# One-2-3-45/One-2-3-45

Measured on NVIDIA H100. Metric: sec/mesh end-to-end (256x256 in), lower is better.
Workload: dtype f16

## Files before the change

### include/o2345.h

```cpp
#ifndef O2345_H_
#define O2345_H_

#include <stddef.h>
#include <stdint.h>

#ifdef __cplusplus
extern "C" {
#endif

#define O2345_OK 0
#define O2345_EINVAL (-1)
#define O2345_ECUDA (-2)
#define O2345_EUNSUPPORTED (-3)

#define O2345_ABI_VERSION 5

typedef void* o2345_stream_t;

int o2345_abi_version(void);
int o2345_last_error(char* buf, size_t n);
int o2345_device_info(int* major, int* minor, int* sms);


#define O2345_SDF_PE 39
#define O2345_SDF_HID 128
#define O2345_SDF_LAT 16
#define O2345_SDF_IN1 144
#define O2345_SDF_PACK_FLOATS (39 * 128 + 128 + 2 * (144 * 128 + 128) + 128 * 144 + 128 * 48)

int o2345_sdf_pack_weights(const float* w0, const float* b0, const float* w1, const float* b1,
                           const float* w2, const float* b2, float* pack, o2345_stream_t stream);

#define O2345_PTS_EXPLICIT 0
#define O2345_PTS_LATTICE 1
#define O2345_PTS_RAYS 2

typedef struct o2345_points {
  int mode;
  const float* pts;
  const float* lin;
  int R;
  const float* rays_o;
  const float* rays_d;
  const float* z;
  int S;
  int z_stride;
} o2345_points;

#define O2345_SDF_FP32 0
#define O2345_SDF_TC_SPLIT 1
int o2345_sdf_query(const o2345_points* src, int64_t n, const float* vol_cl, int D, const float* wpack,
                    const uint8_t* active, float inactive_sdf, int negate, int precision, float* sdf, float* feat,
                    float* latent, float* grad, o2345_stream_t stream);


int o2345_frustum_mask(const float* proj, int V, const float* origin, float voxel_size, int D, int sizeH,
                       int sizeW, int min_views, uint32_t* mask_bits, uint8_t* keep, o2345_stream_t stream);

int64_t o2345_compact_scratch_ints(int64_t n);
int o2345_compact(const uint8_t* flags, int64_t n, int32_t* rows, int32_t* index, int32_t* count,
                  int32_t* scratch, o2345_stream_t stream);

int o2345_costvol_gather(const float* feats_nhwc, int V, int h, int w, int sizeH, int sizeW, const float* proj,
                         const float* origin, float voxel_size, int D, const int32_t* rows, const int32_t* count,
                         int64_t max_rows, const uint32_t* mask_bits, float* cost, o2345_stream_t stream);

int o2345_dense_scatter(const float* feat, const int32_t* rows, const int32_t* count, int64_t max_rows, int D,
                        float* vol_cl, float* vol_cf, float* occ, o2345_stream_t stream);

int o2345_occ_nearest(const o2345_points* src, int64_t n, const float* occ, int D, uint8_t* out,
                      o2345_stream_t stream);


int o2345_sdf_voxels(const float* occ, const float* vol_cl, int D, const float* origin, float voxel_size,
                     const float* wpack, int precision, float* sdf_vol, o2345_stream_t stream);

int o2345_prune_by_sdf(const float* sdf, const float* occ, int D, const float* ladder, int n_ladder, float* scratch,
                       float* minabs, int32_t* counts, o2345_stream_t stream);
int o2345_prune_select(const float* minabs, int64_t n, float threshold, uint8_t* keep, o2345_stream_t stream);
int o2345_clear_flags(const int32_t* rows, const int32_t* idx, int64_t n, uint8_t* flags, o2345_stream_t stream);
int o2345_gather_rows(const int32_t* rows, int64_t n, int D, const float* vol_cf, int C, float* coords, float* feats,
                      o2345_stream_t stream);

int o2345_lod_children(const float* pre_coords, int64_t n, int D1, const uint8_t* frustum_keep, uint8_t* keep,
                       int32_t* parent, int32_t* err_scratch, o2345_stream_t stream);

int o2345_costvol_gather_lod(const float* feats_nhwc, int C, int V, int h, int w, int sizeH, int sizeW, const float* proj,
                             const float* origin, float voxel_size, int D, const int32_t* rows, const int32_t* count,
                             int64_t max_rows, const uint32_t* mask_bits, const int32_t* parent, const float* pre_feats,
                             float* cost, o2345_stream_t stream);


int o2345_sp_coarsen(const int32_t* fine_index, int Ef, const int32_t* fine_rows, const int32_t* fine_count,
                     int64_t max_fine, int Ec, uint8_t* coarse_flags, int32_t* cmin_scratch,
                     o2345_stream_t stream);

int o2345_sp_conv(const float* in_feats, const int32_t* in_index, int Ein, const int32_t* out_rows,
                  const int32_t* out_count, int64_t max_out, int Eout, int mode, const float* kernel, int Cin,
                  int Cout, float* out_raw, double* stats, o2345_stream_t stream);

int o2345_sp_bn_relu(const float* x, const int32_t* count, int64_t max_rows, int C, const double* stats,
                     const float* gamma, const float* beta, float eps, const float* skip, float* out,
                     o2345_stream_t stream);

int o2345_mc_classify(const float* u, int R, float iso, uint8_t* cases, uint8_t* cell_flags, uint8_t* edge_flags,
                      o2345_stream_t stream);
int o2345_mc_vertices(const float* u, int R, float iso, const int32_t* edges, const int32_t* count,
                      int64_t max_verts, double* verts, o2345_stream_t stream);
int64_t o2345_scan_scratch_ints(int64_t n);
int o2345_mc_tri_offsets(const uint8_t* cases, const int32_t* cells, const int32_t* count, int64_t max_cells,
                         const uint8_t* n_tri_table, int32_t* offsets, int32_t* total, int32_t* scratch,
                         o2345_stream_t stream);
int o2345_mc_triangles(const uint8_t* cases, int R, const int32_t* cells, const int32_t* count, int64_t max_cells,
                       const int32_t* tri_offsets, const int8_t* tri_table, const uint8_t* n_tri_table,
                       const int8_t* edge_owner, const int32_t* vert_index, int32_t* tris, o2345_stream_t stream);

typedef struct o2345_view4 {
  float* ptr;
  int64_t sn, sc, sh, sw;
  int c0;
} o2345_view4;

int o2345_conv2d(const float* in, int N, int Cin, int H, int W, const float* weight, const float* bias, int Cout,
                 int K, int stride, int pad, float* out, double* stats, o2345_stream_t stream);
int o2345_abn_apply(const float* x, int N, int C, int H, int W, const double* stats, const float* gamma,
                    const float* beta, float eps, float slope, const o2345_view4* out, o2345_stream_t stream);
int o2345_upsample_bilinear(const float* x, int N, int C, int H, int W, int factor, const float* add,
                            const o2345_view4* out, o2345_stream_t stream);


int o2345_ray_upsample(const float* rays_o, const float* rays_d, int64_t R, const float* z, const float* sdf,
                       int S, float inv_s, const float* occ, int D, const float* u, int n_new, float* new_z,
                       o2345_stream_t stream);
int o2345_ray_merge(const float* z, const float* sdf, int S, const float* new_z, const float* new_sdf, int n_new,
                    int64_t R, float* out_z, float* out_sdf, o2345_stream_t stream);
int o2345_ray_midpoints(const float* rays_o, const float* rays_d, int64_t R, const float* z, int S,
                        float sample_dist, const float* occ, int D, float* mid_z, float* dists, uint8_t* active,
                        o2345_stream_t stream);

#define O2345_MAP_CH 60
#define O2345_RNET_PACK_FLOATS 19664

typedef struct o2345_views {
  int V, H, W;
  const float* maps;
  const float* proj;
  const float* centers;
  float sizeW, sizeH;
} o2345_views;

#define O2345_BLEND_FP32 0
#define O2345_BLEND_TC_FP16 1
int o2345_render_blend(const o2345_points* src, int64_t n, const uint8_t* active, const float* vol_cl,
                       const float* occ, int D, const o2345_views* views, int dir_mode, const float* query_center,
                       const float* dirs, const float* rnet_pack, int precision, float* rgb, int32_t* nvalid,
                       o2345_stream_t stream);

int o2345_ray_composite(const float* rays_d, int64_t R, int S, const float* mid_z, const float* dists,
                        const float* sdf, const float* grad, const float* color, const uint8_t* active,
                        const int32_t* nvalid, float inv_s, float alpha_inter_ratio, int has_background,
                        float background, float* color_out, float* depth_out, float* weights_out, float* cdf_out,
                        float* alpha_out, float* weights_sum_out, uint8_t* color_mask_out, o2345_stream_t stream);

typedef struct {
  const float* bias;
  const void* residual;
  const void* rowbias;
  int64_t rowbias_ld;
  int rows_per_group;
  int act;
  float alpha;
  int out_f32;
  float* colstats;
  int stats_rows_per_group;
} o2345_epilogue;

int o2345_gemm_f16(const void* A, const void* B, void* C, int M, int N, int K, int64_t lda, int64_t ldb,
                   int64_t ldc, int nh, int nb, int64_t stride_a_h, int64_t stride_a_b, int64_t stride_b_h,
                   int64_t stride_b_b, int64_t stride_c_h, int64_t stride_c_b, const o2345_epilogue* ep ,
                   float* splitk_ws, int64_t ws_floats, o2345_stream_t stream);

int o2345_last_trap(char* buf, size_t n);

void o2345_debug_gemm_force(int ctas, int bn, int splits);
void o2345_debug_gemm_persist(int mode, int min_tiles);
void o2345_debug_gemm_model(const float* seven);

void o2345_debug_gemm_trace(long long* device_buf16);

int o2345_conv3x3_f16(const void* x, int B, int H, int W, int C, const void* weight, int N, void* out, int64_t ldc,
                      const o2345_epilogue* ep, float* splitk_ws, int64_t ws_floats, o2345_stream_t stream);

int o2345_conv_up2x_f16(const void* x, int B, int H, int W, int C, const void* weight4, int N, void* out, int64_t ldc,
                        const o2345_epilogue* ep, float* splitk_ws, int64_t ws_floats, o2345_stream_t stream);

int64_t o2345_groupnorm_scratch_floats(int B, int G);
int o2345_groupnorm_stats(const void* x, int B, int HW, int C, int G, float eps, const float* gamma, const float* beta,
                          float* scratch, float* scale, float* shift, o2345_stream_t stream);
int o2345_groupnorm_apply(const void* x, int B, int HW, int C, int G, float eps, const float* gamma, const float* beta, int act,
                          void* out, o2345_stream_t stream);
void o2345_debug_groupnorm_cluster(int cl);
int o2345_norm_act_im2col(const void* x, int B, int H, int W, int C, int ksize, int stride, int upsample, int pad_lo,
                          const float* scale, const float* shift, int act, void* out, o2345_stream_t stream);
int o2345_norm_act_im2col_stats(const void* x, int B, int H, int W, int C, int ksize, int stride, int upsample, int pad_lo,
                                const float* stats_a, int Ca, const float* stats_b, int G, float eps, const float* gamma,
                                const float* beta, int act, void* out, o2345_stream_t stream);
int o2345_layernorm_rows(const void* x, int64_t M, int C, float eps, const float* gamma, const float* beta, void* y,
                         o2345_stream_t stream);
int o2345_softmax_rows(const void* s, int64_t rows, int n, void* p, o2345_stream_t stream);
int o2345_attention_f16(const void* q, const void* k, const void* v, int B, int N, int H, int d, int ld, void* out,
                        int ldo, float scale, o2345_stream_t stream);
int o2345_geglu(const void* x, int64_t M, int I, void* y, o2345_stream_t stream);
int o2345_silu(const void* x, int64_t n, void* y, o2345_stream_t stream);
int o2345_transpose_tokens(const void* x, int B, int N, int C, void* y, o2345_stream_t stream);
int o2345_timestep_embedding(const float* t, int B, int dim, void* out, o2345_stream_t stream);
int o2345_add_channel_bias(void* y, const void* e, int B, int HW, int C, int lde, o2345_stream_t stream);
int o2345_copy_channels(const void* src, int64_t M, int C, void* dst, int ldd, int off, o2345_stream_t stream);
int o2345_nchw_f32_to_cl_f16(const float* x, int B, int C, int HW, void* y, int ldy, int off, o2345_stream_t stream);
int o2345_cl_f16_to_nchw_f32(const void* x, int B, int C, int HW, int ldx, float* y, o2345_stream_t stream);
int o2345_cfg_ddim_update(const float* x, const float* eps, const float* noise, int64_t n, float scale, float a_t,
                          float a_prev, float sigma_t, float sqrt_one_minus_at, float* x_prev, float* pred_x0,
                          o2345_stream_t stream);

int o2345_clip_patches(const float* x, int B, int H, int W, int res, int patch, const float* mean3, const float* std3, int kp,
                       void* out, o2345_stream_t stream);
int o2345_clip_add_positions(void* tok, const float* cls, const float* pos, int B, int N, int d, o2345_stream_t stream);

#ifdef __cplusplus
}
#endif
#endif
```

### one-2-3-45_b200/csrc/gemm_tc.cu

```cuda
#include <cuda.h>
#include <stdlib.h>
#include <cuda_fp16.h>

#include "common.cuh"
#include "wgmma.cuh"

namespace o2345 {
namespace {

constexpr int BM = 128, BK = 64;
constexpr int EPI_WARPS = 8;
constexpr int EPI_THREADS = 32 * EPI_WARPS;
constexpr int GEMM_THREADS = 128 + EPI_THREADS;
constexpr uint64_t WAIT_LIMIT_NS = 4000000000ull;
constexpr int MAX_CLUSTER = 8;
constexpr int RES_PREFETCH = 8;

enum { WAIT_EMPTY = 1, WAIT_FULL = 2 };

struct TrapRecord {
  unsigned long long magic;
  int tag, stage, bx, by, bz, rank, M, N, K, bn, mode, splits, conv;
};
constexpr unsigned long long TRAP_MAGIC = 0x6f32333435545250ull;

__device__ __forceinline__ uint32_t smem_u32(const void* p) { return (uint32_t)__cvta_generic_to_shared(p); }

__device__ __forceinline__ void mbar_init(uint64_t* bar, uint32_t count) {
  asm volatile("mbarrier.init.shared::cta.b64 [%0], %1;" ::"r"(smem_u32(bar)), "r"(count));
}
__device__ __forceinline__ void mbar_expect_tx(uint64_t* bar, uint32_t bytes) {
  asm volatile("mbarrier.arrive.expect_tx.shared::cta.b64 _, [%0], %1;" ::"r"(smem_u32(bar)), "r"(bytes) : "memory");
}
__device__ __forceinline__ void mbar_arrive(uint64_t* bar) {
  asm volatile("mbarrier.arrive.shared::cta.b64 _, [%0];" ::"r"(smem_u32(bar)) : "memory");
}
__device__ __forceinline__ uint32_t mbar_try(uint64_t* bar, uint32_t parity) {
  uint32_t done;
  asm volatile(
      "{\n\t.reg .pred p;\n\t"
      "mbarrier.try_wait.parity.shared::cta.b64 p, [%1], %2;\n\t"
      "selp.u32 %0, 1, 0, p;\n\t}"
      : "=r"(done)
      : "r"(smem_u32(bar)), "r"(parity)
      : "memory");
  return done;
}
__device__ __forceinline__ uint64_t global_ns() {
  uint64_t t;
  asm volatile("mov.u64 %0, %%globaltimer;" : "=l"(t));
  return t;
}
__device__ __forceinline__ void tma_load_2d(void* dst, const CUtensorMap* map, uint64_t* bar, int c0, int c1) {
  asm volatile(
      "cp.async.bulk.tensor.2d.shared::cluster.global.mbarrier::complete_tx::bytes [%0], [%1, {%3, %4}], [%2];"
      ::"r"(smem_u32(dst)), "l"(map), "r"(smem_u32(bar)), "r"(c0), "r"(c1)
      : "memory");
}
__device__ __forceinline__ void tma_load_4d(void* dst, const CUtensorMap* map, uint64_t* bar, int c0, int c1, int c2, int c3) {
  asm volatile(
      "cp.async.bulk.tensor.4d.shared::cluster.global.mbarrier::complete_tx::bytes [%0], [%1, {%3, %4, %5, %6}], [%2];"
      ::"r"(smem_u32(dst)), "l"(map), "r"(smem_u32(bar)), "r"(c0), "r"(c1), "r"(c2), "r"(c3)
      : "memory");
}
__device__ __forceinline__ uint32_t cluster_ctarank() {
  uint32_t r;
  asm volatile("mov.u32 %0, %%cluster_ctarank;" : "=r"(r));
  return r;
}
__device__ __forceinline__ void cluster_sync_all() {
  asm volatile("barrier.cluster.arrive.release.aligned;\n\tbarrier.cluster.wait.acquire.aligned;" ::: "memory");
}
__device__ __forceinline__ void epi_bar() { asm volatile("bar.sync 1, 256;" ::: "memory"); }

__host__ __device__ constexpr int acc_ld(int bn) { return bn + 4; }
__device__ __forceinline__ void acc_ld32(const float* src, uint32_t (&r)[32]) {
#pragma unroll
  for (int i = 0; i < 8; ++i) {
    const float4 v = reinterpret_cast<const float4*>(src)[i];
    r[4 * i] = __float_as_uint(v.x), r[4 * i + 1] = __float_as_uint(v.y), r[4 * i + 2] = __float_as_uint(v.z), r[4 * i + 3] = __float_as_uint(v.w);
  }
}

struct GemmParams {
  int M, N, K;
  int64_t ldc;
  int nh;
  int64_t stride_c_h, stride_c_b;
  const float* bias;
  const __half* rowbias;
  int64_t rowbias_ld;
  int rows_per_group;
  const __half* residual;
  void* C;
  int out_f32;
  int act;
  float alpha;
  int batched;
  int conv, cC, cH, cW, cblocks;
  int ctaps, ctx, cox, coy, up, upa, upb;
  int splits;
  float* ws;
  int persist;
  float* colstats;
  int stats_rpg, stats_groups;
  long long* trace;
  TrapRecord* diag;
  int bn, mode;
};

__device__ __forceinline__ void stamp(const GemmParams& p, int slot) {
  if (p.trace && blockIdx.x == 0 && blockIdx.y == 0 && blockIdx.z == 0) p.trace[slot] = clock64();
}
__device__ __forceinline__ void stamp_ns(const GemmParams& p, int slot, bool any_z = false) {
  if (p.trace && blockIdx.x == 0 && blockIdx.y == 0 && (any_z || blockIdx.z == 0)) p.trace[slot] = (long long)global_ns();
}

__device__ __forceinline__ int64_t out_row(const GemmParams& p, int row) {
  if (!p.up) return row;
  const int x = row % p.cW, t = row / p.cW, y = t % p.cH, b = t / p.cH;
  return ((int64_t)b * (2 * p.cH) + 2 * y + p.upa) * (2 * p.cW) + 2 * x + p.upb;
}

__device__ __noinline__ void wait_timed_out(const GemmParams& p, int tag, int stage) {
  if (p.diag) {
    TrapRecord* d = p.diag;
    d->tag = tag, d->stage = stage, d->bx = blockIdx.x, d->by = blockIdx.y, d->bz = blockIdx.z, d->rank = (int)cluster_ctarank();
    d->M = p.M, d->N = p.N, d->K = p.K, d->bn = p.bn, d->mode = p.mode, d->splits = p.splits, d->conv = p.conv;
    __threadfence_system();
    d->magic = TRAP_MAGIC;
    __threadfence_system();
  }
  __trap();
}
__device__ __forceinline__ void mbar_wait(uint64_t* bar, uint32_t parity, const GemmParams& p, int tag, int stage) {
  if (mbar_try(bar, parity)) return;
  const uint64_t t0 = global_ns();
  uint32_t spins = 0;
  while (!mbar_try(bar, parity))
    if (((++spins) & 255u) == 0 && global_ns() - t0 > WAIT_LIMIT_NS) wait_timed_out(p, tag, stage);
}

__device__ __forceinline__ float gelu_erf(float x) { return 0.5f * x * (1.f + erff(x * 0.70710678118654752f)); }
__device__ __forceinline__ float gelu_erf_fast(float x) {
  const float z = fabsf(x) * 0.70710678118654752f;
  const float t = __fdividef(1.f, fmaf(0.3275911f, z, 1.f));
  const float poly = t * fmaf(t, fmaf(t, fmaf(t, fmaf(t, 1.061405429f, -1.453152027f), 1.421413741f), -0.284496736f), 0.254829592f);
  float e;
  asm("ex2.approx.ftz.f32 %0, %1;" : "=f"(e) : "f"(-z * z * 1.4426950408889634f));
  const float erf_abs = fmaf(-poly, e, 1.f);
  return 0.5f * x * (1.f + copysignf(erf_abs, x));
}
__device__ __forceinline__ float apply_act(float x, int act) {
  if (act == 1) return x / (1.f + __expf(-x));
  if (act == 2) return gelu_erf(x);
  if (act == 4) return x / (1.f + __expf(-1.702f * x));
  return x;
}

__device__ __forceinline__ void store8(const GemmParams& p, int64_t off, const float (&v)[8]) {
  if (p.out_f32) {
    float* o = reinterpret_cast<float*>(p.C) + off;
    *reinterpret_cast<float4*>(o) = make_float4(v[0], v[1], v[2], v[3]);
    *reinterpret_cast<float4*>(o + 4) = make_float4(v[4], v[5], v[6], v[7]);
  } else {
    __half2 h[4];
#pragma unroll
    for (int e = 0; e < 4; ++e) h[e] = __floats2half2_rn(v[2 * e], v[2 * e + 1]);
    *reinterpret_cast<uint4*>(reinterpret_cast<__half*>(p.C) + off) = *reinterpret_cast<uint4*>(h);
  }
}

__device__ __forceinline__ void epilogue_chunk(const GemmParams& p, const uint32_t (&r)[32], int row, int64_t crow, int col0) {
  const __half* rb = p.rowbias ? p.rowbias + (int64_t)(row / p.rows_per_group) * p.rowbias_ld : nullptr;
  if (p.act == 3) {
    if (col0 >= p.N) return;
    float v[16];
#pragma unroll
    for (int e = 0; e < 16; ++e) {
      float a = __uint_as_float(r[e]) * p.alpha, g = __uint_as_float(r[16 + e]) * p.alpha;
      if (p.bias) a += __ldg(p.bias + col0 + e), g += __ldg(p.bias + col0 + 16 + e);
      v[e] = a * gelu_erf(g);
    }
    const int64_t o = crow + (col0 >> 1);
    float lo[8], hi[8];
#pragma unroll
    for (int e = 0; e < 8; ++e) lo[e] = v[e], hi[e] = v[8 + e];
    store8(p, o, lo);
    store8(p, o + 8, hi);
    return;
  }
#pragma unroll
  for (int j = 0; j < 32; j += 8) {
    const int col = col0 + j;
    if (col >= p.N) break;
    float v[8];
    const bool full = col + 8 <= p.N;
    if (full && rb) {
      uint4 q = *reinterpret_cast<const uint4*>(rb + col);
      const __half* h = reinterpret_cast<const __half*>(&q);
#pragma unroll
      for (int e = 0; e < 8; ++e) v[e] = __half2float(h[e]);
    } else {
#pragma unroll
      for (int e = 0; e < 8; ++e) v[e] = (rb && col + e < p.N) ? __half2float(rb[col + e]) : 0.f;
    }
#pragma unroll
    for (int e = 0; e < 8; ++e) {
      float x = fmaf(__uint_as_float(r[j + e]), p.alpha, v[e]);
      if (p.bias && col + e < p.N) x += __ldg(p.bias + col + e);
      v[e] = apply_act(x, p.act);
    }
    if (full && (p.ldc & 7) == 0) {
      if (p.residual) {
        uint4 q = *reinterpret_cast<const uint4*>(p.residual + crow + col);
        const __half* h = reinterpret_cast<const __half*>(&q);
#pragma unroll
        for (int e = 0; e < 8; ++e) v[e] += __half2float(h[e]);
      }
      store8(p, crow + col, v);
    } else {
      for (int e = 0; e < 8 && col + e < p.N; ++e) {
        float x = v[e];
        if (p.residual) x += __half2float(p.residual[crow + col + e]);
        if (p.out_f32) reinterpret_cast<float*>(p.C)[crow + col + e] = x;
        else reinterpret_cast<__half*>(p.C)[crow + col + e] = __float2half_rn(x);
      }
    }
  }
}

__device__ __forceinline__ void splitk_partial(const GemmParams& p, const uint32_t (&r)[32], int split, int row, int col0) {
  float* w = p.ws + ((int64_t)split * p.M + row) * p.N + col0;
  if ((p.N & 3) == 0) {
#pragma unroll
    for (int e = 0; e < 32; e += 4)
      if (col0 + e < p.N)
        __stcg(reinterpret_cast<float4*>(w + e), make_float4(__uint_as_float(r[e]), __uint_as_float(r[e + 1]),
                                                              __uint_as_float(r[e + 2]), __uint_as_float(r[e + 3])));
  } else {
#pragma unroll
    for (int e = 0; e < 32; ++e)
      if (col0 + e < p.N) __stcg(w + e, __uint_as_float(r[e]));
  }
}

template <int BN>
__device__ __forceinline__ void splitk_finalize(const GemmParams& p, int m0, int n0, int z, int te, float* sstat) {
  const bool vec = (p.N % 8) == 0 && (p.ldc % 8) == 0 && (!p.rowbias || (p.rowbias_ld % 8) == 0);
  const int64_t plane = (int64_t)p.M * p.N;
  const bool stats = p.colstats != nullptr && vec && !p.out_f32;
  if (stats) {
    for (int i = te; i < 4 * BN; i += EPI_THREADS) sstat[i] = 0.f;
    epi_bar();
  }
  if (vec) {
    constexpr int PPR = BN / 8;
    constexpr int NP = BM * PPR;
    const int share = (NP + p.splits - 1) / p.splits;
    const int i1 = min(NP, (z + 1) * share);
    constexpr bool FIXED_COLS = (EPI_THREADS % PPR) == 0;
    float bcol[8];
#pragma unroll
    for (int e = 0; e < 8; ++e) bcol[e] = 0.f;
    if (FIXED_COLS && p.bias) {
      const int i0 = z * share + te, col = n0 + (i0 - (i0 / PPR) * PPR) * 8;
      if (col < p.N) {
        const float4 b0 = __ldg(reinterpret_cast<const float4*>(p.bias + col)), b1 = __ldg(reinterpret_cast<const float4*>(p.bias + col + 4));
        bcol[0] = b0.x, bcol[1] = b0.y, bcol[2] = b0.z, bcol[3] = b0.w, bcol[4] = b1.x, bcol[5] = b1.y, bcol[6] = b1.z, bcol[7] = b1.w;
      }
    }
    for (int i = z * share + te; i < i1; i += EPI_THREADS) {
      const int rl = i / PPR, row = m0 + rl, col = n0 + (i - rl * PPR) * 8;
      if (row >= p.M || col >= p.N) continue;
      const int64_t woff = (int64_t)row * p.N + col, o = out_row(p, row) * p.ldc + col;
      uint4 qb = make_uint4(0u, 0u, 0u, 0u), qr = make_uint4(0u, 0u, 0u, 0u);
      if (p.rowbias) qb = *reinterpret_cast<const uint4*>(p.rowbias + (int64_t)(row / p.rows_per_group) * p.rowbias_ld + col);
      if (p.residual) qr = *reinterpret_cast<const uint4*>(p.residual + o);
      if (!FIXED_COLS && p.bias) {
        const float4 b0 = __ldg(reinterpret_cast<const float4*>(p.bias + col)), b1 = __ldg(reinterpret_cast<const float4*>(p.bias + col + 4));
        bcol[0] = b0.x, bcol[1] = b0.y, bcol[2] = b0.z, bcol[3] = b0.w, bcol[4] = b1.x, bcol[5] = b1.y, bcol[6] = b1.z, bcol[7] = b1.w;
      }
      float v[8];
#pragma unroll
      for (int e = 0; e < 8; ++e) v[e] = 0.f;
      for (int s = 0; s < p.splits; s += 4) {
        float4 a[4], b[4];
#pragma unroll
        for (int t = 0; t < 4; ++t) {
          const bool on = s + t < p.splits;
          const float4* w = reinterpret_cast<const float4*>(p.ws + (int64_t)(s + t) * plane + woff);
          a[t] = on ? __ldcg(w) : make_float4(0.f, 0.f, 0.f, 0.f);
          b[t] = on ? __ldcg(w + 1) : make_float4(0.f, 0.f, 0.f, 0.f);
        }
#pragma unroll
        for (int t = 0; t < 4; ++t) {
          v[0] += a[t].x, v[1] += a[t].y, v[2] += a[t].z, v[3] += a[t].w;
          v[4] += b[t].x, v[5] += b[t].y, v[6] += b[t].z, v[7] += b[t].w;
        }
      }
      const __half* hb = reinterpret_cast<const __half*>(&qb);
#pragma unroll
      for (int e = 0; e < 8; ++e) {
        const float x = fmaf(v[e], p.alpha, p.rowbias ? __half2float(hb[e]) : 0.f) + bcol[e];
        v[e] = apply_act(x, p.act);
      }
      if (p.residual) {
        const __half* h = reinterpret_cast<const __half*>(&qr);
#pragma unroll
        for (int e = 0; e < 8; ++e) v[e] += __half2float(h[e]);
      }
      store8(p, o, v);
      if (stats) {
        float* acc = sstat + (row / p.stats_rpg - m0 / p.stats_rpg) * 2 * BN + (col - n0);
#pragma unroll
        for (int e = 0; e < 8; ++e) {
          const float x = __half2float(__float2half_rn(v[e]));
          atomicAdd(acc + e, x), atomicAdd(acc + BN + e, x * x);
        }
      }
    }
    if (stats) {
      epi_bar();
      const int g0 = m0 / p.stats_rpg;
      const int last_row = m0 + BM - 1 < p.M ? m0 + BM - 1 : p.M - 1;
      const int ng = last_row / p.stats_rpg - g0 + 1;
      for (int i = te; i < ng * 2 * BN; i += EPI_THREADS) {
        const int gi = i / (2 * BN), rem = i - gi * 2 * BN, mom = rem / BN, c = rem - mom * BN;
        if (n0 + c < p.N && sstat[i] != 0.f) atomicAdd(p.colstats + ((int64_t)(g0 + gi) * 2 + mom) * p.N + n0 + c, sstat[i]);
      }
    }
    return;
  }
  const int share = (BM * BN + p.splits - 1) / p.splits;
  const int i1 = min(BM * BN, (z + 1) * share);
  for (int i = z * share + te; i < i1; i += EPI_THREADS) {
    const int rl = i / BN, row = m0 + rl, col = n0 + (i - rl * BN);
    if (row >= p.M || col >= p.N) continue;
    float x = 0.f;
    for (int s = 0; s < p.splits; ++s) x += __ldcg(p.ws + (int64_t)s * plane + (int64_t)row * p.N + col);
    x *= p.alpha;
    if (p.rowbias) x += __half2float(p.rowbias[(int64_t)(row / p.rows_per_group) * p.rowbias_ld + col]);
    if (p.bias) x += __ldg(p.bias + col);
    x = apply_act(x, p.act);
    const int64_t o = out_row(p, row) * p.ldc + col;
    if (p.residual) x += __half2float(p.residual[o]);
    if (p.out_f32) reinterpret_cast<float*>(p.C)[o] = x;
    else reinterpret_cast<__half*>(p.C)[o] = __float2half_rn(x);
  }
}

constexpr int EPI_RB_GROUPS = 8;
__host__ __device__ constexpr int epi_smem_bytes(int bn) { return bn * 4 + EPI_RB_GROUPS * bn * 2; }
__host__ __device__ constexpr int col_split(int bn) { return ((bn / 2 + 31) / 32) * 32; }

template <int BN>
__device__ __forceinline__ void epilogue_preload(const GemmParams& p, int m0, int n0, float* sbias, __half* srb, int te) {
  for (int i = te; i < BN; i += EPI_THREADS) sbias[i] = (p.bias && n0 + i < p.N) ? __ldg(p.bias + n0 + i) : 0.f;
  if (p.rowbias) {
    const int g0 = m0 / p.rows_per_group;
    const int last = (m0 + BM - 1 < p.M ? m0 + BM - 1 : p.M - 1) / p.rows_per_group;
    const int ng = last - g0 + 1;
    if (ng >= 1 && ng <= EPI_RB_GROUPS)
      for (int i = te; i < ng * BN; i += EPI_THREADS) {
        const int gi = i / BN, c = i - gi * BN;
        srb[i] = (n0 + c < p.N) ? p.rowbias[(int64_t)(g0 + gi) * p.rowbias_ld + n0 + c] : __float2half(0.f);
      }
  }
  epi_bar();
}

template <int ACT>
__device__ __forceinline__ float act_fn(float x) {
  if (ACT == 1) return __fdividef(x, 1.f + __expf(-x));
  if (ACT == 2) return gelu_erf(x);
  if (ACT == 4) return __fdividef(x, 1.f + __expf(-1.702f * x));
  return x;
}

template <int ACT>
__device__ __forceinline__ void stage_rows(const GemmParams& p, const float* acc_row, uint8_t* mine, int n0, int c_lo, int c_hi,
                                           const float* sbias, const __half* rb, bool rb_smem) {
#pragma unroll 1
  for (int c0 = c_lo; c0 < c_hi; c0 += 32) {
    if (n0 + c0 >= p.N) break;
    uint32_t r[32];
    acc_ld32(acc_row + c0, r);
    if (ACT == 3) {
      __half2 h[8];
#pragma unroll
      for (int e = 0; e < 16; e += 2) {
        float a0 = fmaf(__uint_as_float(r[e]), p.alpha, sbias[c0 + e]), a1 = fmaf(__uint_as_float(r[e + 1]), p.alpha, sbias[c0 + e + 1]);
        float g0 = fmaf(__uint_as_float(r[16 + e]), p.alpha, sbias[c0 + 16 + e]);
        float g1 = fmaf(__uint_as_float(r[17 + e]), p.alpha, sbias[c0 + 17 + e]);
        h[e >> 1] = __floats2half2_rn(a0 * gelu_erf_fast(g0), a1 * gelu_erf_fast(g1));
      }
      uint4* d = reinterpret_cast<uint4*>(mine + (c0 - c_lo));
      d[0] = reinterpret_cast<uint4*>(h)[0], d[1] = reinterpret_cast<uint4*>(h)[1];
    } else {
#pragma unroll
      for (int j = 0; j < 32; j += 8) {
        float v[8];
        const float4 b0 = *reinterpret_cast<const float4*>(sbias + c0 + j), b1 = *reinterpret_cast<const float4*>(sbias + c0 + j + 4);
        v[0] = b0.x, v[1] = b0.y, v[2] = b0.z, v[3] = b0.w, v[4] = b1.x, v[5] = b1.y, v[6] = b1.z, v[7] = b1.w;
        if (rb && (rb_smem || n0 + c0 + j + 8 <= p.N)) {
          uint4 q = *reinterpret_cast<const uint4*>(rb + c0 + j);
          const __half* hq = reinterpret_cast<const __half*>(&q);
#pragma unroll
          for (int e = 0; e < 8; ++e) v[e] += __half2float(hq[e]);
        }
        __half2 h[4];
#pragma unroll
        for (int e = 0; e < 8; e += 2) {
          float x0 = fmaf(__uint_as_float(r[j + e]), p.alpha, v[e]), x1 = fmaf(__uint_as_float(r[j + e + 1]), p.alpha, v[e + 1]);
          h[e >> 1] = __floats2half2_rn(act_fn<ACT>(x0), act_fn<ACT>(x1));
        }
        *reinterpret_cast<uint4*>(mine + (c0 - c_lo + j) * 2) = *reinterpret_cast<uint4*>(h);
      }
    }
  }
}

struct WarpOut {
  int outc, stride, ppr, total, ocol0, nout;
};
template <int MODE>
__device__ __forceinline__ WarpOut warp_out(const GemmParams& p, int n0, int c_lo, int c_hi) {
  constexpr bool geglu = MODE == 1;
  WarpOut g;
  g.outc = geglu ? (c_hi - c_lo) >> 1 : (c_hi - c_lo);
  g.stride = g.outc * 2 + 16;
  g.ppr = g.outc >> 3;
  g.total = 32 * g.ppr;
  g.ocol0 = geglu ? (n0 + c_lo) >> 1 : n0 + c_lo;
  g.nout = geglu ? p.N >> 1 : p.N;
  return g;
}

__device__ __forceinline__ void prefetch_residual(const GemmParams& p, const WarpOut& g, int lane, int row0,
                                                  uint4 (&resq)[RES_PREFETCH]) {
#pragma unroll
  for (int u = 0; u < RES_PREFETCH; ++u) {
    resq[u] = make_uint4(0u, 0u, 0u, 0u);
    const int pp = lane + 32 * u;
    if (p.residual && pp < g.total) {
      const int rl = pp / g.ppr, ci = pp - rl * g.ppr;
      const int grow = row0 + rl, col = g.ocol0 + ci * 8;
      if (grow < p.M && col < g.nout) resq[u] = *reinterpret_cast<const uint4*>(p.residual + out_row(p, grow) * p.ldc + col);
    }
  }
}

__device__ __forceinline__ uint4 add_h8(uint4 v, uint4 q) {
  __half2* a = reinterpret_cast<__half2*>(&v);
  const __half2* b = reinterpret_cast<const __half2*>(&q);
#pragma unroll
  for (int e = 0; e < 4; ++e) {
    float2 fa = __half22float2(a[e]), fb = __half22float2(b[e]);
    a[e] = __floats2half2_rn(fa.x + fb.x, fa.y + fb.y);
  }
  return v;
}

template <int BN, int MODE>
__device__ __forceinline__ void epilogue_staged(const GemmParams& p, const WarpOut& g, const float* acc_row, uint8_t* slab, int lane,
                                                int m0, int row0, int n0, int c_lo, int c_hi, const float* sbias, const __half* srb,
                                                const uint4 (&resq)[RES_PREFETCH]) {
  const int row = row0 + lane;
  const __half* rb = nullptr;
  bool rb_smem = false;
  if (MODE != 1 && p.rowbias) {
    const int rr = row < p.M ? row : p.M - 1;
    const int g0 = m0 / p.rows_per_group, last = (m0 + BM - 1 < p.M ? m0 + BM - 1 : p.M - 1) / p.rows_per_group;
    rb_smem = last - g0 + 1 <= EPI_RB_GROUPS;
    rb = rb_smem ? srb + (rr / p.rows_per_group - g0) * BN : p.rowbias + (int64_t)(rr / p.rows_per_group) * p.rowbias_ld + n0;
  }
  uint8_t* mine = slab + lane * g.stride;
  if (MODE == 0) {
    stage_rows<0>(p, acc_row, mine, n0, c_lo, c_hi, sbias, rb, rb_smem);
  } else if (MODE == 1) {
    stage_rows<3>(p, acc_row, mine, n0, c_lo, c_hi, sbias, rb, rb_smem);
  } else {
    switch (p.act) {
      case 1: stage_rows<1>(p, acc_row, mine, n0, c_lo, c_hi, sbias, rb, rb_smem); break;
      case 2: stage_rows<2>(p, acc_row, mine, n0, c_lo, c_hi, sbias, rb, rb_smem); break;
      default: stage_rows<4>(p, acc_row, mine, n0, c_lo, c_hi, sbias, rb, rb_smem); break;
    }
  }
  __syncwarp();
  __half* C = reinterpret_cast<__half*>(p.C);
#pragma unroll
  for (int u = 0; u < RES_PREFETCH; ++u) {
    const int pp = lane + 32 * u;
    if (pp < g.total) {
      const int rl = pp / g.ppr, ci = pp - rl * g.ppr;
      const int grow = row0 + rl, col = g.ocol0 + ci * 8;
      if (grow < p.M && col < g.nout) {
        uint4 v = *reinterpret_cast<const uint4*>(slab + rl * g.stride + ci * 16);
        if (p.residual) {
          v = add_h8(v, resq[u]);
          if (p.colstats) *reinterpret_cast<uint4*>(slab + rl * g.stride + ci * 16) = v;
        }
        *reinterpret_cast<uint4*>(C + out_row(p, grow) * p.ldc + col) = v;
      }
    }
  }
  constexpr int UN = 4;
  for (int base = lane + 32 * RES_PREFETCH; base < g.total; base += 32 * UN) {
    uint4 v[UN], q[UN];
    int64_t o[UN];
    bool ok[UN];
#pragma unroll
    for (int u = 0; u < UN; ++u) {
      const int pp = base + 32 * u;
      const int rl = pp / g.ppr, ci = pp - rl * g.ppr;
      const int grow = row0 + rl, col = g.ocol0 + ci * 8;
      ok[u] = pp < g.total && grow < p.M && col < g.nout;
      o[u] = out_row(p, grow) * p.ldc + col;
      if (ok[u]) {
        v[u] = *reinterpret_cast<const uint4*>(slab + rl * g.stride + ci * 16);
        if (p.residual) q[u] = *reinterpret_cast<const uint4*>(p.residual + o[u]);
      }
    }
#pragma unroll
    for (int u = 0; u < UN; ++u) {
      if (!ok[u]) continue;
      if (p.residual) {
        v[u] = add_h8(v[u], q[u]);
        if (p.colstats) {
          const int pp = base + 32 * u;
          const int rl = pp / g.ppr, ci = pp - rl * g.ppr;
          *reinterpret_cast<uint4*>(slab + rl * g.stride + ci * 16) = v[u];
        }
      }
      *reinterpret_cast<uint4*>(C + o[u]) = v[u];
    }
  }
  if (MODE == 0 && p.colstats) {
    __syncwarp();
    const int nrows = p.M - row0 < 32 ? p.M - row0 : 32;
    if (nrows > 0) {
      float* ssum = p.colstats + (int64_t)(row0 / p.stats_rpg) * 2 * g.nout;
      for (int cp = lane; 2 * cp < g.outc; cp += 32) {
        const int col = g.ocol0 + 2 * cp;
        if (col >= g.nout) break;
        float s0 = 0.f, s1 = 0.f, q0 = 0.f, q1 = 0.f;
        if (nrows == 32) {
#pragma unroll 8
          for (int r = 0; r < 32; ++r) {
            const float2 f = __half22float2(*reinterpret_cast<const __half2*>(slab + r * g.stride + cp * 4));
            s0 += f.x, s1 += f.y, q0 = fmaf(f.x, f.x, q0), q1 = fmaf(f.y, f.y, q1);
          }
        } else {
          for (int r = 0; r < nrows; ++r) {
            const float2 f = __half22float2(*reinterpret_cast<const __half2*>(slab + r * g.stride + cp * 4));
            s0 += f.x, s1 += f.y, q0 = fmaf(f.x, f.x, q0), q1 = fmaf(f.y, f.y, q1);
          }
        }
        atomicAdd(ssum + col, s0), atomicAdd(ssum + col + 1, s1);
        atomicAdd(ssum + g.nout + col, q0), atomicAdd(ssum + g.nout + col + 1, q1);
      }
    }
  }
}

__host__ __device__ constexpr int epi_slab_bytes(int bn) { return EPI_WARPS * 32 * (col_split(bn) * 2 + 16); }
constexpr int smem_bytes(int bn, int stages) {
  return stages * (BM * BK * 2 + bn * BK * 2) + epi_slab_bytes(bn) + 2 * stages * 8 + 16 + epi_smem_bytes(bn) + 1024;
}

template <int BN>
__device__ __forceinline__ void produce_stage(const GemmParams& p, const CUtensorMap* tmA, const CUtensorMap* tmB, uint8_t* a_dst,
                                              uint8_t* b_dst, uint64_t* full_bar, int kb, int m0, int n0, int bz) {
  mbar_expect_tx(full_bar, BM * BK * 2 + BN * BK * 2);
  if (p.conv) {
    const int tap = kb / p.cblocks, c0 = (kb - tap * p.cblocks) * BK;
    const int x0 = m0 % p.cW, y0 = (m0 / p.cW) % p.cH, b0 = m0 / (p.cW * p.cH);
    tma_load_4d(a_dst, tmA, full_bar, c0, x0 + tap % p.ctx + p.cox, y0 + tap / p.ctx + p.coy, b0);
    tma_load_2d(b_dst, tmB, full_bar, tap * p.cC + c0, n0);
  } else if (p.batched) {
    tma_load_4d(a_dst, tmA, full_bar, kb * BK, m0, bz % p.nh, bz / p.nh);
    tma_load_4d(b_dst, tmB, full_bar, kb * BK, n0, bz % p.nh, bz / p.nh);
  } else {
    tma_load_2d(a_dst, tmA, full_bar, kb * BK, m0);
    tma_load_2d(b_dst, tmB, full_bar, kb * BK, n0);
  }
}

template <int BN>
__device__ __forceinline__ void acc_store(float* acc, const float (&d)[BN / 2], int row0, int t) {
  const int r = row0 + 16 * (t >> 5) + ((t & 31) >> 2), c = 2 * (t & 3);
#pragma unroll
  for (int j = 0; j < BN / 8; ++j) {
    *reinterpret_cast<float2*>(acc + r * acc_ld(BN) + 8 * j + c) = make_float2(d[4 * j], d[4 * j + 1]);
    *reinterpret_cast<float2*>(acc + (r + 8) * acc_ld(BN) + 8 * j + c) = make_float2(d[4 * j + 2], d[4 * j + 3]);
  }
}

template <int BN, int STAGES, int MODE>
__global__ void __launch_bounds__(GEMM_THREADS, 1)
gemm_tc_kernel(const __grid_constant__ CUtensorMap tmA, const __grid_constant__ CUtensorMap tmB, const __grid_constant__ GemmParams p) {
  extern __shared__ __align__(1024) uint8_t smem_raw[];
  uint8_t* smem = reinterpret_cast<uint8_t*>((reinterpret_cast<uintptr_t>(smem_raw) + 1023) & ~(uintptr_t)1023);
  constexpr int A_BYTES = BM * BK * 2, B_BYTES = BN * BK * 2;
  static_assert(B_BYTES % 1024 == 0, "stage bases must stay 1024-byte aligned for SWIZZLE_128B");
  static_assert(BN % 32 == 0 && BN >= 64 && BN <= 256, "tile width: a multiple of 32 (GEGLU chunks, 32-column epilogue reads)");
  static_assert(BM * acc_ld(BN) * 4 <= STAGES * (A_BYTES + B_BYTES), "the accumulator tile must fit in the operand ring");
  constexpr int CSPLIT = col_split(BN);
  uint8_t* sA = smem;
  uint8_t* sB = smem + STAGES * A_BYTES;
  uint8_t* slabs = sB + STAGES * B_BYTES;
  uint64_t* full = reinterpret_cast<uint64_t*>(slabs + epi_slab_bytes(BN));
  uint64_t* empty = full + STAGES;
  float* sbias = reinterpret_cast<float*>((reinterpret_cast<uintptr_t>(empty + STAGES) + 15) & ~(uintptr_t)15);
  __half* srb = reinterpret_cast<__half*>(sbias + BN);
  float* acc = reinterpret_cast<float*>(smem);

  const int warp = threadIdx.x >> 5, lane = threadIdx.x & 31;
  if (threadIdx.x == 0) stamp(p, 0), stamp_ns(p, 16);
  const int bz = blockIdx.z;
  const int nk = p.conv ? p.ctaps * p.cblocks : (p.K + BK - 1) / BK;
  const bool split = MODE == 3 && p.splits > 1;
  int kb0 = 0, kb1 = nk;
  if (split) {
    kb0 = (int)((int64_t)nk * bz / p.splits);
    kb1 = (int)((int64_t)nk * (bz + 1) / p.splits);
  }

  if (threadIdx.x == 0) {
    asm volatile("prefetch.tensormap [%0];" ::"l"(&tmA) : "memory");
    asm volatile("prefetch.tensormap [%0];" ::"l"(&tmB) : "memory");
    for (int s = 0; s < STAGES; ++s) mbar_init(full + s, 1), mbar_init(empty + s, 2);
    asm volatile("fence.mbarrier_init.release.cluster;" ::: "memory");
    asm volatile("fence.proxy.async.shared::cta;" ::: "memory");
  }
  __syncthreads();
  pdl_wait();
  pdl_trigger();
  if (threadIdx.x == 0) stamp(p, 1);

  const int tiles_m = (p.M + BM - 1) / BM, tiles = tiles_m * ((p.N + BN - 1) / BN);
  const bool persist = MODE != 3 && p.persist;
  uint32_t cnt = 0;
  for (int t = persist ? blockIdx.x : blockIdx.y * tiles_m + blockIdx.x; t < tiles; t += persist ? gridDim.x : tiles) {
  const int m0 = (t % tiles_m) * BM, n0 = (t / tiles_m) * BN;
  if (warp < 4) {
    if (threadIdx.x == 0) {
      asm volatile("fence.proxy.async.shared::cta;" ::: "memory");
      for (int kb = kb0; kb < kb1; ++kb) {
        const uint32_t c = cnt + (kb - kb0);
        const int s = c % STAGES;
        const uint32_t ph = (c / STAGES) & 1;
        mbar_wait(empty + s, ph ^ 1, p, WAIT_EMPTY, s);
        produce_stage<BN>(p, &tmA, &tmB, sA + s * A_BYTES, sB + s * B_BYTES, full + s, kb, m0, n0, bz);
        if (kb == kb0) stamp(p, 2);
      }
      stamp(p, 3);
    }
    __syncwarp();
  } else {
    const int wg = (warp >> 2) - 1, e = warp - 4, quarter = e & 3, te = threadIdx.x - 128;
    const int c_lo = e < 4 ? 0 : CSPLIT, c_hi = e < 4 ? CSPLIT : BN;
    const int row0 = m0 + quarter * 32;
    if (MODE != 3) epilogue_preload<BN>(p, m0, n0, sbias, srb, te);
    {
      float d[BN / 2];
#pragma unroll
      for (int i = 0; i < BN / 2; ++i) d[i] = 0.f;
      for (int kb = kb0; kb < kb1; ++kb) {
        const uint32_t c = cnt + (kb - kb0);
        const int s = c % STAGES;
        const uint32_t ph = (c / STAGES) & 1;
        mbar_wait(full + s, ph, p, WAIT_FULL, s);
        if (kb == kb0 && te == 0) stamp(p, 4);
        const uint32_t a0 = smem_u32(sA + s * A_BYTES) + wg * (64 * 128), b0 = smem_u32(sB + s * B_BYTES);
        wg::fence();
#pragma unroll
        for (int k = 0; k < BK / 16; ++k)
          wg::mma_f16<BN>(d, wg::desc_sw128(a0 + k * 32), wg::desc_sw128(b0 + k * 32), 1);
        wg::commit();
        wg::wait<1>();
        if (kb > kb0 && (threadIdx.x & 127) == 0) mbar_arrive(empty + (c - 1) % STAGES);
      }
      wg::wait<0>();
      if ((threadIdx.x & 127) == 0) mbar_arrive(empty + (cnt + kb1 - kb0 - 1) % STAGES);
      if (te == 0) stamp(p, 5);
      epi_bar();
      acc_store<BN>(acc, d, 64 * wg, threadIdx.x & 127);
    }
    epi_bar();
    if (te == 0) stamp(p, 6);
    const float* acc_row = acc + (quarter * 32 + lane) * acc_ld(BN);
    if (MODE != 3) {
      const WarpOut g = warp_out<MODE>(p, n0, c_lo, c_hi);
      uint4 resq[RES_PREFETCH];
      prefetch_residual(p, g, lane, row0, resq);
      epilogue_staged<BN, MODE>(p, g, acc_row, slabs + e * 32 * (CSPLIT * 2 + 16), lane, m0, row0, n0, c_lo, c_hi, sbias, srb, resq);
    } else {
      const int row = row0 + lane;
      if (split) {
        if (te == 0) stamp_ns(p, 17);
#pragma unroll 1
        for (int c0 = c_lo; c0 < c_hi; c0 += 32) {
          uint32_t r[32];
          acc_ld32(acc_row + c0, r);
          if (row < p.M) splitk_partial(p, r, bz, row, n0 + c0);
        }
        if (te == 0) stamp_ns(p, 18);
      } else {
        const int64_t crow = (p.batched ? (int64_t)(bz % p.nh) * p.stride_c_h + (int64_t)(bz / p.nh) * p.stride_c_b : 0) +
                             out_row(p, row < p.M ? row : 0) * p.ldc;
#pragma unroll 1
        for (int c0 = c_lo; c0 < c_hi; c0 += 32) {
          uint32_t r[32];
          acc_ld32(acc_row + c0, r);
          if (row < p.M) epilogue_chunk(p, r, row, crow, n0 + c0);
        }
      }
    }
    if (te == 0) stamp(p, 7);
  }
  cnt += kb1 - kb0;
  __syncthreads();
  }
  if (split) {
    cluster_sync_all();
    if (warp >= 4) {
      if (threadIdx.x == 128) stamp_ns(p, 21, true);
      splitk_finalize<BN>(p, blockIdx.x * BM, blockIdx.y * BN, bz, threadIdx.x - 128, reinterpret_cast<float*>(smem));
      if (threadIdx.x == 128) stamp_ns(p, 22, true);
    }
  }
  if (threadIdx.x == 0) stamp(p, 8);
}

typedef CUresult (*EncodeTiledFn)(CUtensorMap*, CUtensorMapDataType, cuuint32_t, void*, const cuuint64_t*, const cuuint64_t*,
                                  const cuuint32_t*, const cuuint32_t*, CUtensorMapInterleave, CUtensorMapSwizzle,
                                  CUtensorMapL2promotion, CUtensorMapFloatOOBfill);

EncodeTiledFn encode_fn() {
  static EncodeTiledFn fn = nullptr;
  if (!fn) {
    void* p = nullptr;
    cudaDriverEntryPointQueryResult q;
    if (cudaGetDriverEntryPoint("cuTensorMapEncodeTiled", &p, cudaEnableDefault, &q) == cudaSuccess && q == cudaDriverEntryPointSuccess)
      fn = reinterpret_cast<EncodeTiledFn>(p);
  }
  return fn;
}

int make_map(CUtensorMap* m, const void* ptr, int64_t rows, int64_t K, int64_t ld, int nh, int nb, int64_t sh, int64_t sb,
             int box_rows) {
  EncodeTiledFn fn = encode_fn();
  if (!fn) { set_error("cuTensorMapEncodeTiled entry point not available"); return O2345_ECUDA; }
  cuuint64_t dims[4] = {(cuuint64_t)K, (cuuint64_t)rows, (cuuint64_t)(nh > 0 ? nh : 1), (cuuint64_t)(nb > 0 ? nb : 1)};
  cuuint64_t strides[3] = {(cuuint64_t)ld * 2, (cuuint64_t)sh * 2, (cuuint64_t)sb * 2};
  cuuint32_t box[4] = {(cuuint32_t)BK, (cuuint32_t)box_rows, 1, 1};
  cuuint32_t estr[4] = {1, 1, 1, 1};
  int rank = nh > 0 ? 4 : 2;
  CUresult r = fn(m, CU_TENSOR_MAP_DATA_TYPE_FLOAT16, rank, const_cast<void*>(ptr), dims, strides, box, estr,
                  CU_TENSOR_MAP_INTERLEAVE_NONE, CU_TENSOR_MAP_SWIZZLE_128B, CU_TENSOR_MAP_L2_PROMOTION_L2_256B,
                  CU_TENSOR_MAP_FLOAT_OOB_FILL_NONE);
  if (r != CUDA_SUCCESS) { set_error("cuTensorMapEncodeTiled failed with %d (rows=%lld K=%lld ld=%lld)", (int)r, (long long)rows, (long long)K, (long long)ld); return O2345_ECUDA; }
  return O2345_OK;
}

TrapRecord* g_diag = nullptr;
bool g_diag_tried = false;
TrapRecord* diag_buffer(cudaStream_t st) {
  if (!g_diag_tried) {
    cudaStreamCaptureStatus cs = cudaStreamCaptureStatusNone;
    if (cudaStreamIsCapturing(st, &cs) != cudaSuccess || cs != cudaStreamCaptureStatusNone) {
      cudaGetLastError();
      return g_diag;
    }
    g_diag_tried = true;
    void* h = nullptr;
    if (cudaHostAlloc(&h, sizeof(TrapRecord), cudaHostAllocMapped | cudaHostAllocPortable) == cudaSuccess) {
      memset(h, 0, sizeof(TrapRecord));
      g_diag = reinterpret_cast<TrapRecord*>(h);
    } else {
      cudaGetLastError();
    }
  }
  return g_diag;
}

struct Config {
  int bn, splits;
  int persist;
};

int g_force[3] = {-1, 0, 0};
int g_persist = 0;
int g_persist_min_tiles = 0;
void read_force_env() {
  if (g_force[0] >= 0) return;
  g_force[0] = g_force[1] = g_force[2] = 0;
  const char* e = getenv("O2345_GEMM_FORCE");
  if (e) sscanf(e, "%d,%d,%d", &g_force[0], &g_force[1], &g_force[2]);
}

float g_model[7] = {40.f, 0.5f, 6300.f, 5.f, 3.f, 4.f, 1.f};
float predict_us(int M, int N, int nk, int bn, int splits) {
  const float bw_sm = g_model[0], alpha = g_model[1], cap = g_model[2], fixed = g_model[3], epi = g_model[4], so0 = g_model[5],
              so1 = g_model[6], cyc_per_us = 1750.f;
  const int tiles = cdiv(M, BM) * cdiv(N, bn);
  const int n = tiles * splits;
  const int kb = cdiv(nk, splits);
  const float bytes_cta = (float)kb * (float)(BM * BK * 2 + bn * BK * 2);
  const int sms = sm_count();
  const int rounds = cdiv(n, sms);
  float f = (float)(n - sms) / (float)sms;
  f = f < 0.f ? 0.f : (f > 1.f ? 1.f : f);
  const float t_sm = (float)rounds * bytes_cta / (bw_sm * (1.f + alpha * f));
  const float t_fabric = (float)n * bytes_cta / cap;
  const float t_mma = (float)rounds * (float)kb * 4.f * (float)bn;
  float t = t_sm > t_fabric ? t_sm : t_fabric;
  if (t_mma > t) t = t_mma;
  float us = fixed + t / cyc_per_us + epi * (float)bn / 160.f * (float)cdiv(n, sms);
  if (splits > 1) us += so0 + so1 * (float)splits * (float)bn / 128.f;
  return us;
}

Config pick_config(const GemmParams& p, int nk, bool can_split, int64_t ws_floats) {
  read_force_env();
  Config c;
  const int M = p.M, N = p.N;
  c.persist = 0;
  if (p.batched) {
    c.bn = N <= 64 ? 64 : 128, c.splits = 1;
    return c;
  }
  static const int kBn[4] = {64, 128, 160, 256};
  static const int kSplits[6] = {1, 2, 3, 4, 6, 8};
  const bool split_ok = can_split && p.act != 3 && p.ws && 2 * (int64_t)M * N <= ws_floats;
  const int max_planes = split_ok ? (int)(ws_floats / ((int64_t)M * N)) : 1;
  float best = 1e30f;
  c.bn = 128, c.splits = 1;
  for (int bi = 0; bi < 4; ++bi) {
    const int bn = kBn[bi];
    if (bn > 64 && N <= 64) continue;
    if (g_force[1] > 0 && bn != g_force[1]) continue;
    for (int si = 0; si < 6; ++si) {
      const int sp = kSplits[si];
      if (g_force[2] > 0 && sp != (g_force[2] > nk ? nk : g_force[2])) continue;
      if (sp > 1 && (!split_ok || sp > max_planes || sp > MAX_CLUSTER || nk / sp < 3)) continue;
      const float us = predict_us(M, N, nk, bn, sp);
      if (us < best) best = us, c.bn = bn, c.splits = sp;
    }
  }
  if (best > 1e29f) {
    c.bn = (g_force[1] == 64 || g_force[1] == 128 || g_force[1] == 160 || g_force[1] == 256) ? g_force[1] : 128;
    c.splits = 1;
  }
  const int tiles = cdiv(M, BM) * cdiv(N, c.bn);
  const int min_tiles = g_persist_min_tiles > 0 ? g_persist_min_tiles : 4 * sm_count();
  c.persist = c.splits == 1 && (g_persist == 1 || (g_persist == 0 && tiles >= min_tiles));
  return c;
}

int pick_mode(const GemmParams& p, const Config& c) {
  const int nout = p.act == 3 ? p.N / 2 : p.N;
  const bool staged = !p.out_f32 && c.splits <= 1 && !p.batched && (nout % 8) == 0 && (p.ldc % 8) == 0 && ((uintptr_t)p.C % 16) == 0 &&
                      (!p.residual || ((uintptr_t)p.residual % 16) == 0);
  if (!staged) return 3;
  return p.act == 0 ? 0 : (p.act == 3 ? 1 : 2);
}

long long* g_trace = nullptr;

template <int BN, int STAGES, int MODE>
int launch(const CUtensorMap& a, const CUtensorMap& b, GemmParams p, int batch, int persist, cudaStream_t st) {
  constexpr int SMEM = smem_bytes(BN, STAGES);
  static_assert(SMEM <= 227 * 1024, "one CTA per SM");
  static PerDeviceOnce attr;
  if (attr.need())
    O2345_CUDA(cudaFuncSetAttribute(gemm_tc_kernel<BN, STAGES, MODE>, cudaFuncAttributeMaxDynamicSharedMemorySize, SMEM));
  p.bn = BN, p.mode = MODE;
  p.diag = diag_buffer(st);
  const int splits = (MODE == 3 && batch == 0 && p.splits > 1) ? p.splits : 1;
  p.splits = splits;
  dim3 grid(cdiv(p.M, BM), cdiv(p.N, BN), batch > 0 ? batch : splits);
  p.persist = MODE != 3 && batch == 0 && splits == 1 && persist;
  if (p.persist) {
    const int tiles = (int)grid.x * (int)grid.y;
    grid = dim3(tiles < sm_count() ? tiles : sm_count(), 1, 1);
  }
  O2345_CUDA(launch_pdl_cluster(gemm_tc_kernel<BN, STAGES, MODE>, grid, dim3(GEMM_THREADS), (size_t)SMEM, st, 1, splits, a, b, p));
  O2345_LAUNCH_CHECK();
  return O2345_OK;
}

template <int BN, int STAGES>
int launch_mode(int mode, const CUtensorMap& a, const CUtensorMap& b, const GemmParams& p, int batch, int persist, cudaStream_t st) {
  switch (mode) {
    case 0: return launch<BN, STAGES, 0>(a, b, p, batch, persist, st);
    case 1: return launch<BN, STAGES, 1>(a, b, p, batch, persist, st);
    case 2: return launch<BN, STAGES, 2>(a, b, p, batch, persist, st);
    default: return launch<BN, STAGES, 3>(a, b, p, batch, persist, st);
  }
}

int dispatch(const Config& c, int mode, const CUtensorMap& a, const CUtensorMap& b, const GemmParams& p, int batch, cudaStream_t st) {
  if (p.colstats && mode == 3 && c.splits <= 1) {
    set_error("o2345_gemm_f16: column statistics need the staged fp16 epilogue (16-byte aligned C / residual) or split-K");
    return O2345_EUNSUPPORTED;
  }
  if (c.bn == 64) return launch_mode<64, 6>(mode, a, b, p, batch, c.persist, st);
  if (c.bn == 128) return launch_mode<128, 5>(mode, a, b, p, batch, c.persist, st);
  if (c.bn == 160) return launch_mode<160, 4>(mode, a, b, p, batch, c.persist, st);
  return launch_mode<256, 3>(mode, a, b, p, batch, c.persist, st);
}

int fill_epilogue(GemmParams& p, const o2345_epilogue* ep, int M, int N, int64_t ldc) {
  p.bias = nullptr, p.rowbias = nullptr, p.rowbias_ld = 0, p.rows_per_group = 1, p.residual = nullptr;
  p.out_f32 = 0, p.act = 0, p.alpha = 1.f, p.trace = g_trace;
  p.colstats = nullptr, p.stats_rpg = 1, p.stats_groups = 0;
  p.diag = nullptr, p.bn = p.mode = 0;
  if (!ep) return O2345_OK;
  O2345_CHECK_ARG(ep->act >= 0 && ep->act <= 4, "unknown activation");
  O2345_CHECK_ARG(!ep->rowbias || (ep->rows_per_group > 0 && (ep->rowbias_ld % 8) == 0 && ((uintptr_t)ep->rowbias % 16) == 0),
                  "row bias: rows_per_group > 0, 16-byte aligned, row stride a multiple of 8");
  O2345_CHECK_ARG(ep->act != 3 || ((N % 32) == 0 && (ldc % 8) == 0 && !ep->residual && !ep->rowbias),
                  "GEGLU epilogue: N must be a multiple of 32, ldc of 8, no residual / row bias");
  p.bias = ep->bias, p.rowbias = reinterpret_cast<const __half*>(ep->rowbias), p.rowbias_ld = ep->rowbias_ld;
  p.rows_per_group = ep->rowbias ? ep->rows_per_group : 1;
  p.residual = reinterpret_cast<const __half*>(ep->residual), p.out_f32 = ep->out_f32, p.act = ep->act, p.alpha = ep->alpha;
  if (ep->colstats) {
    O2345_CHECK_ARG(ep->act == 0 && !ep->out_f32 && (N % 8) == 0 && (ldc % 8) == 0,
                    "column statistics: fp16 output without activation, N and ldc multiples of 8");
    O2345_CHECK_ARG(ep->stats_rows_per_group > 0 && ((ep->stats_rows_per_group % 128) == 0 || ep->stats_rows_per_group == 64),
                    "column statistics: rows per group must be 64 or a multiple of 128");
    p.colstats = ep->colstats, p.stats_rpg = ep->stats_rows_per_group, p.stats_groups = cdiv(M, ep->stats_rows_per_group);
  }
  return O2345_OK;
}

void set_workspace(GemmParams& p, float* ws, int64_t ws_floats) { p.ws = ws_floats > 0 ? ws : nullptr; }

}
}

using namespace o2345;

extern "C" void o2345_debug_gemm_trace(long long* device_buf16) { g_trace = device_buf16; }

extern "C" void o2345_debug_gemm_force(int ctas, int bn, int splits) {
  read_force_env();
  g_force[0] = ctas, g_force[1] = bn, g_force[2] = splits;
}


extern "C" void o2345_debug_gemm_persist(int mode, int min_tiles) { g_persist = mode, g_persist_min_tiles = min_tiles; }

extern "C" void o2345_debug_gemm_model(const float* seven) {
  for (int i = 0; i < 7; ++i) g_model[i] = seven[i];
}

extern "C" int o2345_last_trap(char* buf, size_t n) {
  if (!buf || n == 0) return O2345_EINVAL;
  buf[0] = 0;
  const TrapRecord* d = g_diag;
  if (!d || d->magic != TRAP_MAGIC) return 0;
  static const char* names[] = {"?", "empty (producer waiting for the MMA to free a stage)", "full (MMA issuer waiting for TMA bytes)",
                                };
  snprintf(buf, n,
           "gemm_tc_kernel<BN=%d, MODE=%d> M=%d N=%d K=%d conv=%d splits=%d: CTA (%d,%d,%d) rank %d gave up after 4 s "
           "on barrier '%s' stage %d",
           d->bn, d->mode, d->M, d->N, d->K, d->conv, d->splits, d->bx, d->by, d->bz, d->rank,
           names[d->tag >= 1 && d->tag <= 2 ? d->tag : 0], d->stage);
  return 1;
}

namespace o2345 {
namespace {
int conv_launch(const void* x, int B, int H, int W, int C, const void* weight, int N, void* out, int64_t ldc, const o2345_epilogue* ep,
                float* splitk_ws, int64_t ws_floats, int taps, int tx, int ox, int oy, int up, int upa, int upb, cudaStream_t st) {
  EncodeTiledFn fn = encode_fn();
  if (!fn) { set_error("cuTensorMapEncodeTiled entry point not available"); return O2345_ECUDA; }
  const int tw = W >= 128 ? 128 : W;
  const int th = W >= 128 ? 1 : (128 / W < H ? 128 / W : H);
  const int tb = 128 / (tw * th);
  CUtensorMap ma, mb;
  {
    cuuint64_t dims[4] = {(cuuint64_t)C, (cuuint64_t)W, (cuuint64_t)H, (cuuint64_t)B};
    cuuint64_t strides[3] = {(cuuint64_t)C * 2, (cuuint64_t)W * C * 2, (cuuint64_t)H * W * C * 2};
    cuuint32_t box[4] = {(cuuint32_t)BK, (cuuint32_t)tw, (cuuint32_t)th, (cuuint32_t)tb};
    cuuint32_t estr[4] = {1, 1, 1, 1};
    CUresult r = fn(&ma, CU_TENSOR_MAP_DATA_TYPE_FLOAT16, 4, const_cast<void*>(x), dims, strides, box, estr,
                    CU_TENSOR_MAP_INTERLEAVE_NONE, CU_TENSOR_MAP_SWIZZLE_128B, CU_TENSOR_MAP_L2_PROMOTION_L2_256B,
                    CU_TENSOR_MAP_FLOAT_OOB_FILL_NONE);
    if (r != CUDA_SUCCESS) { set_error("cuTensorMapEncodeTiled (conv activation) failed with %d", (int)r); return O2345_ECUDA; }
  }
  GemmParams p;
  p.M = B * H * W, p.N = N, p.K = taps * C, p.ldc = ldc, p.nh = 1, p.stride_c_h = 0, p.stride_c_b = 0, p.C = out;
  int rc = fill_epilogue(p, ep, p.M, N, ldc);
  if (rc) return rc;
  p.batched = 0, p.conv = 1, p.cC = C, p.cH = H, p.cW = W, p.cblocks = (C + BK - 1) / BK;
  p.ctaps = taps, p.ctx = tx, p.cox = ox, p.coy = oy, p.up = up, p.upa = upa, p.upb = upb;
  set_workspace(p, splitk_ws, ws_floats);
  const Config c = pick_config(p, taps * p.cblocks, true, ws_floats);
  p.splits = c.splits;
  rc = make_map(&mb, weight, N, taps * (int64_t)C, taps * (int64_t)C, 0, 0, 0, 0, c.bn);
  if (rc) return rc;
  return dispatch(c, pick_mode(p, c), ma, mb, p, 0, st);
}

bool conv_tiles(int H, int W) {
  return (W % 128) == 0 || ((128 % W) == 0 && (((int64_t)H * W >= 128 && (H % (128 / W)) == 0) || ((int64_t)H * W < 128 && (128 % (H * W)) == 0)));
}
}
}

extern "C" int o2345_conv3x3_f16(const void* x, int B, int H, int W, int C, const void* weight, int N, void* out, int64_t ldc,
                                 const o2345_epilogue* ep, float* splitk_ws, int64_t ws_floats, o2345_stream_t stream) {
  O2345_CHECK_ARG(x && weight && out, "null pointer");
  O2345_CHECK_ARG(B > 0 && H > 0 && W > 0 && C > 0 && (C % 8) == 0 && N > 0, "bad sizes (C must be a multiple of 8)");
  O2345_CHECK_ARG(conv_tiles(H, W),
                  "implicit 3x3 conv: the image must tile into 128-pixel boxes (W % 128 == 0, or 128 % W == 0 with "
                  "H % (128 / W) == 0, or 128 % (H * W) == 0)");
  O2345_CHECK_ARG(((uintptr_t)x % 16) == 0 && ((uintptr_t)weight % 16) == 0, "operands must be 16-byte aligned");
  return conv_launch(x, B, H, W, C, weight, N, out, ldc, ep, splitk_ws, ws_floats, 9, 3, -1, -1, 0, 0, 0, (cudaStream_t)stream);
}

extern "C" int o2345_conv_up2x_f16(const void* x, int B, int H, int W, int C, const void* weight4, int N, void* out, int64_t ldc,
                                   const o2345_epilogue* ep, float* splitk_ws, int64_t ws_floats, o2345_stream_t stream) {
  O2345_CHECK_ARG(x && weight4 && out, "null pointer");
  O2345_CHECK_ARG(B > 0 && H > 0 && W > 0 && C > 0 && (C % 8) == 0 && N > 0, "bad sizes (C must be a multiple of 8)");
  O2345_CHECK_ARG(conv_tiles(H, W), "up-sampling conv: the LOW-resolution image must tile into 128-pixel boxes (see o2345_conv3x3_f16)");
  O2345_CHECK_ARG(((uintptr_t)x % 16) == 0 && ((uintptr_t)weight4 % 16) == 0, "operands must be 16-byte aligned");
  O2345_CHECK_ARG(!ep || (!ep->residual && !ep->colstats && !ep->rowbias && ep->act != 3),
                  "up-sampling conv: bias / activation epilogues only (no residual, row bias, statistics, GEGLU)");
  O2345_CHECK_ARG((int64_t)B * 4 * H * W < (1ll << 31), "output rows must fit 31 bits");
  const __half* w = reinterpret_cast<const __half*>(weight4);
  for (int ph = 0; ph < 4; ++ph) {
    const int a = ph >> 1, b = ph & 1;
    int rc = conv_launch(x, B, H, W, C, w + (int64_t)ph * N * 4 * C, N, out, ldc, ep, splitk_ws, ws_floats, 4, 2, b - 1, a - 1, 1, a, b,
                         (cudaStream_t)stream);
    if (rc) return rc;
  }
  return O2345_OK;
}

extern "C" int o2345_gemm_f16(const void* A, const void* B, void* C, int M, int N, int K, int64_t lda, int64_t ldb,
                              int64_t ldc, int nh, int nb, int64_t stride_a_h, int64_t stride_a_b, int64_t stride_b_h,
                              int64_t stride_b_b, int64_t stride_c_h, int64_t stride_c_b, const o2345_epilogue* ep,
                              float* splitk_ws, int64_t ws_floats, o2345_stream_t stream) {
  O2345_CHECK_ARG(A && B && C, "null pointer");
  O2345_CHECK_ARG(M > 0 && N > 0 && K > 0 && nh >= 0 && (nh == 0 || nb >= 1), "bad sizes");
  O2345_CHECK_ARG((lda % 8) == 0 && (ldb % 8) == 0, "row strides of A and B must be multiples of 8 fp16 (16 bytes) for TMA");
  O2345_CHECK_ARG(((uintptr_t)A % 16) == 0 && ((uintptr_t)B % 16) == 0, "A and B must be 16-byte aligned");
  O2345_CHECK_ARG(nh == 0 || ((stride_a_h % 8) == 0 && (stride_a_b % 8) == 0 && (stride_b_h % 8) == 0 && (stride_b_b % 8) == 0),
                  "batch strides must be multiples of 8 fp16");
  GemmParams p;
  p.M = M, p.N = N, p.K = K, p.ldc = ldc, p.nh = nh > 0 ? nh : 1, p.stride_c_h = stride_c_h, p.stride_c_b = stride_c_b, p.C = C;
  int rc = fill_epilogue(p, ep, M, N, ldc);
  if (rc) return rc;
  O2345_CHECK_ARG(nh == 0 || (!p.rowbias && p.act != 3), "row bias / GEGLU are not available in batched mode");
  p.batched = nh > 0 ? 1 : 0;
  p.conv = 0, p.cC = p.cH = p.cW = p.cblocks = 0;
  p.ctaps = p.ctx = p.cox = p.coy = p.up = p.upa = p.upb = 0;
  set_workspace(p, splitk_ws, ws_floats);
  cudaStream_t st = (cudaStream_t)stream;
  const Config c = pick_config(p, cdiv(K, BK), nh == 0, ws_floats);
  p.splits = c.splits;
  CUtensorMap ma, mb;
  rc = make_map(&ma, A, M, K, lda, nh, nb, stride_a_h, stride_a_b, BM);
  if (rc) return rc;
  rc = make_map(&mb, B, N, K, ldb, nh, nb, stride_b_h, stride_b_b, c.bn);
  if (rc) return rc;
  return dispatch(c, pick_mode(p, c), ma, mb, p, nh > 0 ? nh * nb : 0, st);
}
```

### one-2-3-45_b200/o2345/_lib.py

```python
from __future__ import annotations

import ctypes as C
import functools
import os

HERE = os.path.dirname(os.path.abspath(__file__))
LIB_PATH = os.environ.get("O2345_LIB") or os.path.join(os.path.dirname(HERE), "lib", "libo2345_sm90.so")

c_fp = C.c_void_p
c_i64 = C.c_int64


class Points(C.Structure):
    _fields_ = [("mode", C.c_int), ("pts", c_fp), ("lin", c_fp), ("R", C.c_int), ("rays_o", c_fp),
                ("rays_d", c_fp), ("z", c_fp), ("S", C.c_int), ("z_stride", C.c_int)]


class View4(C.Structure):
    _fields_ = [("ptr", c_fp), ("sn", c_i64), ("sc", c_i64), ("sh", c_i64), ("sw", c_i64), ("c0", C.c_int)]


class Views(C.Structure):
    _fields_ = [("V", C.c_int), ("H", C.c_int), ("W", C.c_int), ("maps", c_fp), ("proj", c_fp),
                ("centers", c_fp), ("sizeW", C.c_float), ("sizeH", C.c_float)]


class Epilogue(C.Structure):
    _fields_ = [("bias", c_fp), ("residual", c_fp), ("rowbias", c_fp), ("rowbias_ld", c_i64), ("rows_per_group", C.c_int),
                ("act", C.c_int), ("alpha", C.c_float), ("out_f32", C.c_int), ("colstats", c_fp), ("stats_rows_per_group", C.c_int)]


PTS_EXPLICIT, PTS_LATTICE, PTS_RAYS = 0, 1, 2
BLEND_FP32, BLEND_TC_FP16 = 0, 1
SDF_FP32, SDF_TC_SPLIT = 0, 1
SDF_PACK_FLOATS = 39 * 128 + 128 + 2 * (144 * 128 + 128) + 128 * 144 + 128 * 48
RNET_PACK_FLOATS = 19664
MAP_CH = 60

_SIGS = {
    "o2345_abi_version": (C.c_int, []),
    "o2345_last_error": (C.c_int, [C.c_char_p, C.c_size_t]),
    "o2345_device_info": (C.c_int, [C.POINTER(C.c_int)] * 3),
    "o2345_sdf_pack_weights": (C.c_int, [c_fp] * 7 + [c_fp]),
    "o2345_sdf_query": (C.c_int, [C.POINTER(Points), c_i64, c_fp, C.c_int, c_fp, c_fp, C.c_float, C.c_int, C.c_int,
                                  c_fp, c_fp, c_fp, c_fp, c_fp]),
    "o2345_frustum_mask": (C.c_int, [c_fp, C.c_int, c_fp, C.c_float, C.c_int, C.c_int, C.c_int, C.c_int, c_fp,
                                     c_fp, c_fp]),
    "o2345_compact_scratch_ints": (c_i64, [c_i64]),
    "o2345_compact": (C.c_int, [c_fp, c_i64, c_fp, c_fp, c_fp, c_fp, c_fp]),
    "o2345_costvol_gather": (C.c_int, [c_fp, C.c_int, C.c_int, C.c_int, C.c_int, C.c_int, c_fp, c_fp, C.c_float,
                                       C.c_int, c_fp, c_fp, c_i64, c_fp, c_fp, c_fp]),
    "o2345_dense_scatter": (C.c_int, [c_fp, c_fp, c_fp, c_i64, C.c_int, c_fp, c_fp, c_fp, c_fp]),
    "o2345_sdf_voxels": (C.c_int, [c_fp, c_fp, C.c_int, c_fp, C.c_float, c_fp, C.c_int, c_fp, c_fp]),
    "o2345_prune_by_sdf": (C.c_int, [c_fp, c_fp, C.c_int, C.POINTER(C.c_float), C.c_int, c_fp, c_fp, c_fp, c_fp]),
    "o2345_prune_select": (C.c_int, [c_fp, c_i64, C.c_float, c_fp, c_fp]),
    "o2345_clear_flags": (C.c_int, [c_fp, c_fp, c_i64, c_fp, c_fp]),
    "o2345_gather_rows": (C.c_int, [c_fp, c_i64, C.c_int, c_fp, C.c_int, c_fp, c_fp, c_fp]),
    "o2345_lod_children": (C.c_int, [c_fp, c_i64, C.c_int, c_fp, c_fp, c_fp, c_fp, c_fp]),
    "o2345_costvol_gather_lod": (C.c_int, [c_fp, C.c_int, C.c_int, C.c_int, C.c_int, C.c_int, C.c_int, c_fp, c_fp, C.c_float,
                                           C.c_int, c_fp, c_fp, c_i64, c_fp, c_fp, c_fp, c_fp, c_fp]),
    "o2345_occ_nearest": (C.c_int, [C.POINTER(Points), c_i64, c_fp, C.c_int, c_fp, c_fp]),
    "o2345_sp_coarsen": (C.c_int, [c_fp, C.c_int, c_fp, c_fp, c_i64, C.c_int, c_fp, c_fp, c_fp]),
    "o2345_sp_conv": (C.c_int, [c_fp, c_fp, C.c_int, c_fp, c_fp, c_i64, C.c_int, C.c_int, c_fp, C.c_int, C.c_int,
                                c_fp, c_fp, c_fp]),
    "o2345_sp_bn_relu": (C.c_int, [c_fp, c_fp, c_i64, C.c_int, c_fp, c_fp, c_fp, C.c_float, c_fp, c_fp, c_fp]),
    "o2345_mc_classify": (C.c_int, [c_fp, C.c_int, C.c_float, c_fp, c_fp, c_fp, c_fp]),
    "o2345_mc_vertices": (C.c_int, [c_fp, C.c_int, C.c_float, c_fp, c_fp, c_i64, c_fp, c_fp]),
    "o2345_scan_scratch_ints": (c_i64, [c_i64]),
    "o2345_mc_tri_offsets": (C.c_int, [c_fp, c_fp, c_fp, c_i64, c_fp, c_fp, c_fp, c_fp, c_fp]),
    "o2345_mc_triangles": (C.c_int, [c_fp, C.c_int, c_fp, c_fp, c_i64, c_fp, c_fp, c_fp, c_fp, c_fp, c_fp, c_fp]),
    "o2345_conv2d": (C.c_int, [c_fp, C.c_int, C.c_int, C.c_int, C.c_int, c_fp, c_fp, C.c_int, C.c_int, C.c_int,
                               C.c_int, c_fp, c_fp, c_fp]),
    "o2345_abn_apply": (C.c_int, [c_fp, C.c_int, C.c_int, C.c_int, C.c_int, c_fp, c_fp, c_fp, C.c_float, C.c_float,
                                  C.POINTER(View4), c_fp]),
    "o2345_upsample_bilinear": (C.c_int, [c_fp, C.c_int, C.c_int, C.c_int, C.c_int, C.c_int, c_fp,
                                          C.POINTER(View4), c_fp]),
    "o2345_ray_upsample": (C.c_int, [c_fp, c_fp, c_i64, c_fp, c_fp, C.c_int, C.c_float, c_fp, C.c_int, c_fp,
                                     C.c_int, c_fp, c_fp]),
    "o2345_ray_merge": (C.c_int, [c_fp, c_fp, C.c_int, c_fp, c_fp, C.c_int, c_i64, c_fp, c_fp, c_fp]),
    "o2345_ray_midpoints": (C.c_int, [c_fp, c_fp, c_i64, c_fp, C.c_int, C.c_float, c_fp, C.c_int, c_fp, c_fp,
                                      c_fp, c_fp]),
    "o2345_render_blend": (C.c_int, [C.POINTER(Points), c_i64, c_fp, c_fp, c_fp, C.c_int, C.POINTER(Views),
                                     C.c_int, c_fp, c_fp, c_fp, C.c_int, c_fp, c_fp, c_fp]),
    "o2345_gemm_f16": (C.c_int, [c_fp, c_fp, c_fp, C.c_int, C.c_int, C.c_int, c_i64, c_i64, c_i64, C.c_int, C.c_int,
                                 c_i64, c_i64, c_i64, c_i64, c_i64, c_i64, C.POINTER(Epilogue), c_fp, c_i64, c_fp]),
    "o2345_debug_gemm_trace": (None, [c_fp]),
    "o2345_debug_gemm_force": (None, [C.c_int, C.c_int, C.c_int]),
    "o2345_debug_gemm_persist": (None, [C.c_int, C.c_int]),
    "o2345_debug_groupnorm_cluster": (None, [C.c_int]),
    "o2345_debug_gemm_model": (None, [C.POINTER(C.c_float)]),
    "o2345_last_trap": (C.c_int, [C.c_char_p, C.c_size_t]),
    "o2345_conv3x3_f16": (C.c_int, [c_fp, C.c_int, C.c_int, C.c_int, C.c_int, c_fp, C.c_int, c_fp, c_i64,
                                    C.POINTER(Epilogue), c_fp, c_i64, c_fp]),
    "o2345_conv_up2x_f16": (C.c_int, [c_fp, C.c_int, C.c_int, C.c_int, C.c_int, c_fp, C.c_int, c_fp, c_i64,
                                      C.POINTER(Epilogue), c_fp, c_i64, c_fp]),
    "o2345_groupnorm_scratch_floats": (c_i64, [C.c_int, C.c_int]),
    "o2345_groupnorm_stats": (C.c_int, [c_fp, C.c_int, C.c_int, C.c_int, C.c_int, C.c_float, c_fp, c_fp, c_fp, c_fp, c_fp,
                                        c_fp]),
    "o2345_groupnorm_apply": (C.c_int, [c_fp, C.c_int, C.c_int, C.c_int, C.c_int, C.c_float, c_fp, c_fp, C.c_int, c_fp, c_fp]),
    "o2345_norm_act_im2col": (C.c_int, [c_fp, C.c_int, C.c_int, C.c_int, C.c_int, C.c_int, C.c_int, C.c_int, C.c_int, c_fp, c_fp,
                                        C.c_int, c_fp, c_fp]),
    "o2345_norm_act_im2col_stats": (C.c_int, [c_fp, C.c_int, C.c_int, C.c_int, C.c_int, C.c_int, C.c_int, C.c_int, C.c_int, c_fp, C.c_int,
                                              c_fp, C.c_int, C.c_float, c_fp, c_fp, C.c_int, c_fp, c_fp]),
    "o2345_layernorm_rows": (C.c_int, [c_fp, c_i64, C.c_int, C.c_float, c_fp, c_fp, c_fp, c_fp]),
    "o2345_softmax_rows": (C.c_int, [c_fp, c_i64, C.c_int, c_fp, c_fp]),
    "o2345_attention_f16": (C.c_int, [c_fp, c_fp, c_fp, C.c_int, C.c_int, C.c_int, C.c_int, C.c_int, c_fp, C.c_int,
                                      C.c_float, c_fp]),
    "o2345_geglu": (C.c_int, [c_fp, c_i64, C.c_int, c_fp, c_fp]),
    "o2345_silu": (C.c_int, [c_fp, c_i64, c_fp, c_fp]),
    "o2345_transpose_tokens": (C.c_int, [c_fp, C.c_int, C.c_int, C.c_int, c_fp, c_fp]),
    "o2345_timestep_embedding": (C.c_int, [c_fp, C.c_int, C.c_int, c_fp, c_fp]),
    "o2345_add_channel_bias": (C.c_int, [c_fp, c_fp, C.c_int, C.c_int, C.c_int, C.c_int, c_fp]),
    "o2345_copy_channels": (C.c_int, [c_fp, c_i64, C.c_int, c_fp, C.c_int, C.c_int, c_fp]),
    "o2345_nchw_f32_to_cl_f16": (C.c_int, [c_fp, C.c_int, C.c_int, C.c_int, c_fp, C.c_int, C.c_int, c_fp]),
    "o2345_cl_f16_to_nchw_f32": (C.c_int, [c_fp, C.c_int, C.c_int, C.c_int, C.c_int, c_fp, c_fp]),
    "o2345_cfg_ddim_update": (C.c_int, [c_fp, c_fp, c_fp, c_i64, C.c_float, C.c_float, C.c_float, C.c_float, C.c_float,
                                        c_fp, c_fp, c_fp]),
    "o2345_clip_patches": (C.c_int, [c_fp, C.c_int, C.c_int, C.c_int, C.c_int, C.c_int, C.POINTER(C.c_float), C.POINTER(C.c_float),
                                     C.c_int, c_fp, c_fp]),
    "o2345_clip_add_positions": (C.c_int, [c_fp, c_fp, c_fp, C.c_int, C.c_int, C.c_int, c_fp]),
    "o2345_ray_composite": (C.c_int, [c_fp, c_i64, C.c_int, c_fp, c_fp, c_fp, c_fp, c_fp, c_fp, c_fp, C.c_float,
                                      C.c_float, C.c_int, C.c_float, c_fp, c_fp, c_fp, c_fp, c_fp, c_fp, c_fp, c_fp]),
}

EXPORTED = tuple(_SIGS)
ABI_VERSION = 5
_lib = None


class O2345Error(RuntimeError):
    pass


def load():
    global _lib
    if _lib is None:
        if not os.path.exists(LIB_PATH):
            raise O2345Error(f"{LIB_PATH} is missing: run `python one-2-3-45_b200/build.py` "
                             "(there is no CPU or PyTorch fallback for this path)")
        lib = C.CDLL(LIB_PATH)
        for name, (res, args) in _SIGS.items():
            fn = getattr(lib, name)
            fn.restype, fn.argtypes = res, args
        if lib.o2345_abi_version() != ABI_VERSION:
            raise O2345Error(f"{LIB_PATH} has ABI version {lib.o2345_abi_version()}, this binding expects {ABI_VERSION}: "
                             "rebuild with `python one-2-3-45_b200/build.py`")
        _lib = lib
    return _lib


def last_trap() -> str:
    buf = C.create_string_buffer(512)
    return buf.value.decode(errors="replace") if load().o2345_last_trap(buf, 512) == 1 else ""


def last_error() -> str:
    buf = C.create_string_buffer(512)
    load().o2345_last_error(buf, 512)
    return buf.value.decode(errors="replace")


_KERNELS_PER_CALL = {"o2345_compact": 3, "o2345_prune_by_sdf": 3, "o2345_sp_coarsen": 3, "o2345_mc_tri_offsets": 4, "o2345_conv_up2x_f16": 4}
_launches = 0


def reset_launches():
    global _launches
    _launches = 0


def add_launches(n: int):
    global _launches
    _launches += n


def launches() -> int:
    return _launches


def call(name, *args):
    global _launches
    rc = getattr(load(), name)(*args)
    if rc != 0:
        raise O2345Error(f"{name} failed with {rc}: {last_error()}")
    _launches += _KERNELS_PER_CALL.get(name, 1)
    return rc


def inference_only(fn):
    import torch

    @functools.wraps(fn)
    def wrap(self, *args, **kwargs):
        if torch.is_grad_enabled() and any(p.requires_grad for p in self.parameters()):
            raise RuntimeError(f"o2345 {type(self).__name__}.{fn.__name__} is inference-only: call it under torch.no_grad() or "
                               "freeze the parameters (requires_grad_(False)); training stays with the reference")
        with torch.no_grad():
            return fn(self, *args, **kwargs)
    return wrap
```

Baseline: 2.761.

## Add 256-row GEMM tiles with register reallocation and N-fastest tile order

Adds a 256-row tile variant of the warp-specialized wgmma GEMM. Each consumer warpgroup issues two 128-row MMAs per K-step against a shared B tile, so the B operand is reused across more rows and the epilogue runs twice per tile. Producer and consumer warps now rebalance registers with setmaxnreg, a new option walks tiles with N fastest, and the cost model and config picker can choose the tall tile for both convs and GEMMs. In exchange it brings more register pressure (two accumulator sets), fewer pipeline stages (3) and more template instantiations, and the per-tile loops are restructured separately for producer and consumer.

```diff
diff --git a/include/o2345.h b/include/o2345.h
--- a/include/o2345.h
+++ b/include/o2345.h
@@ -13,7 +13,7 @@
 #define O2345_ECUDA (-2)
 #define O2345_EUNSUPPORTED (-3)
 
-#define O2345_ABI_VERSION 5
+#define O2345_ABI_VERSION 6
 
 typedef void* o2345_stream_t;
 
@@ -182,7 +182,7 @@
 
 int o2345_last_trap(char* buf, size_t n);
 
-void o2345_debug_gemm_force(int ctas, int bn, int splits);
+void o2345_debug_gemm_force(int bm, int bn, int splits);
 void o2345_debug_gemm_persist(int mode, int min_tiles);
 void o2345_debug_gemm_model(const float* seven);
 
diff --git a/one-2-3-45_b200/csrc/gemm_tc.cu b/one-2-3-45_b200/csrc/gemm_tc.cu
--- a/one-2-3-45_b200/csrc/gemm_tc.cu
+++ b/one-2-3-45_b200/csrc/gemm_tc.cu
@@ -8,7 +8,9 @@
 namespace o2345 {
 namespace {
 
-constexpr int BM = 128, BK = 64;
+constexpr int BK = 64;
+constexpr int EPI_ROWS = 128;
+constexpr int PRODUCER_REGS = 40, CONSUMER_REGS = 232;
 constexpr int EPI_WARPS = 8;
 constexpr int EPI_THREADS = 32 * EPI_WARPS;
 constexpr int GEMM_THREADS = 128 + EPI_THREADS;
@@ -20,7 +22,7 @@
 
 struct TrapRecord {
   unsigned long long magic;
-  int tag, stage, bx, by, bz, rank, M, N, K, bn, mode, splits, conv;
+  int tag, stage, bx, by, bz, rank, M, N, K, bm, bn, mode, splits, conv;
 };
 constexpr unsigned long long TRAP_MAGIC = 0x6f32333435545250ull;
 
@@ -72,6 +74,10 @@
   asm volatile("barrier.cluster.arrive.release.aligned;\n\tbarrier.cluster.wait.acquire.aligned;" ::: "memory");
 }
 __device__ __forceinline__ void epi_bar() { asm volatile("bar.sync 1, 256;" ::: "memory"); }
+template <int R>
+__device__ __forceinline__ void reg_dealloc() { asm volatile("setmaxnreg.dec.sync.aligned.u32 %0;" ::"n"(R)); }
+template <int R>
+__device__ __forceinline__ void reg_alloc() { asm volatile("setmaxnreg.inc.sync.aligned.u32 %0;" ::"n"(R)); }
 
 __host__ __device__ constexpr int acc_ld(int bn) { return bn + 4; }
 __device__ __forceinline__ void acc_ld32(const float* src, uint32_t (&r)[32]) {
@@ -102,11 +108,12 @@
   int splits;
   float* ws;
   int persist;
+  int n_fastest;
   float* colstats;
   int stats_rpg, stats_groups;
   long long* trace;
   TrapRecord* diag;
-  int bn, mode;
+  int bm, bn, mode;
 };
 
 __device__ __forceinline__ void stamp(const GemmParams& p, int slot) {
@@ -126,7 +133,7 @@
   if (p.diag) {
     TrapRecord* d = p.diag;
     d->tag = tag, d->stage = stage, d->bx = blockIdx.x, d->by = blockIdx.y, d->bz = blockIdx.z, d->rank = (int)cluster_ctarank();
-    d->M = p.M, d->N = p.N, d->K = p.K, d->bn = p.bn, d->mode = p.mode, d->splits = p.splits, d->conv = p.conv;
+    d->M = p.M, d->N = p.N, d->K = p.K, d->bm = p.bm, d->bn = p.bn, d->mode = p.mode, d->splits = p.splits, d->conv = p.conv;
     __threadfence_system();
     d->magic = TRAP_MAGIC;
     __threadfence_system();
@@ -247,6 +254,7 @@
 
 template <int BN>
 __device__ __forceinline__ void splitk_finalize(const GemmParams& p, int m0, int n0, int z, int te, float* sstat) {
+  constexpr int BM = 128;
   const bool vec = (p.N % 8) == 0 && (p.ldc % 8) == 0 && (!p.rowbias || (p.rowbias_ld % 8) == 0);
   const int64_t plane = (int64_t)p.M * p.N;
   const bool stats = p.colstats != nullptr && vec && !p.out_f32;
@@ -350,18 +358,18 @@
   }
 }
 
-constexpr int EPI_RB_GROUPS = 8;
-__host__ __device__ constexpr int epi_smem_bytes(int bn) { return bn * 4 + EPI_RB_GROUPS * bn * 2; }
+__host__ __device__ constexpr int epi_rb_groups(int bm) { return 8 * bm / 128; }
+__host__ __device__ constexpr int epi_smem_bytes(int bm, int bn) { return bn * 4 + epi_rb_groups(bm) * bn * 2; }
 __host__ __device__ constexpr int col_split(int bn) { return ((bn / 2 + 31) / 32) * 32; }
 
-template <int BN>
+template <int BM, int BN>
 __device__ __forceinline__ void epilogue_preload(const GemmParams& p, int m0, int n0, float* sbias, __half* srb, int te) {
   for (int i = te; i < BN; i += EPI_THREADS) sbias[i] = (p.bias && n0 + i < p.N) ? __ldg(p.bias + n0 + i) : 0.f;
   if (p.rowbias) {
     const int g0 = m0 / p.rows_per_group;
     const int last = (m0 + BM - 1 < p.M ? m0 + BM - 1 : p.M - 1) / p.rows_per_group;
     const int ng = last - g0 + 1;
-    if (ng >= 1 && ng <= EPI_RB_GROUPS)
+    if (ng >= 1 && ng <= epi_rb_groups(BM))
       for (int i = te; i < ng * BN; i += EPI_THREADS) {
         const int gi = i / BN, c = i - gi * BN;
         srb[i] = (n0 + c < p.N) ? p.rowbias[(int64_t)(g0 + gi) * p.rowbias_ld + n0 + c] : __float2half(0.f);
@@ -462,7 +470,7 @@
   return v;
 }
 
-template <int BN, int MODE>
+template <int BM, int BN, int MODE>
 __device__ __forceinline__ void epilogue_staged(const GemmParams& p, const WarpOut& g, const float* acc_row, uint8_t* slab, int lane,
                                                 int m0, int row0, int n0, int c_lo, int c_hi, const float* sbias, const __half* srb,
                                                 const uint4 (&resq)[RES_PREFETCH]) {
@@ -472,7 +480,7 @@
   if (MODE != 1 && p.rowbias) {
     const int rr = row < p.M ? row : p.M - 1;
     const int g0 = m0 / p.rows_per_group, last = (m0 + BM - 1 < p.M ? m0 + BM - 1 : p.M - 1) / p.rows_per_group;
-    rb_smem = last - g0 + 1 <= EPI_RB_GROUPS;
+    rb_smem = last - g0 + 1 <= epi_rb_groups(BM);
     rb = rb_smem ? srb + (rr / p.rows_per_group - g0) * BN : p.rowbias + (int64_t)(rr / p.rows_per_group) * p.rowbias_ld + n0;
   }
   uint8_t* mine = slab + lane * g.stride;
@@ -565,11 +573,11 @@
 }
 
 __host__ __device__ constexpr int epi_slab_bytes(int bn) { return EPI_WARPS * 32 * (col_split(bn) * 2 + 16); }
-constexpr int smem_bytes(int bn, int stages) {
-  return stages * (BM * BK * 2 + bn * BK * 2) + epi_slab_bytes(bn) + 2 * stages * 8 + 16 + epi_smem_bytes(bn) + 1024;
-}
-
-template <int BN>
+constexpr int smem_bytes(int bm, int bn, int stages) {
+  return stages * (bm * BK * 2 + bn * BK * 2) + epi_slab_bytes(bn) + 2 * stages * 8 + 16 + epi_smem_bytes(bm, bn) + 1024;
+}
+
+template <int BM, int BN>
 __device__ __forceinline__ void produce_stage(const GemmParams& p, const CUtensorMap* tmA, const CUtensorMap* tmB, uint8_t* a_dst,
                                               uint8_t* b_dst, uint64_t* full_bar, int kb, int m0, int n0, int bz) {
   mbar_expect_tx(full_bar, BM * BK * 2 + BN * BK * 2);
@@ -597,15 +605,17 @@
   }
 }
 
-template <int BN, int STAGES, int MODE>
+template <int BM, int BN, int STAGES, int MODE>
 __global__ void __launch_bounds__(GEMM_THREADS, 1)
 gemm_tc_kernel(const __grid_constant__ CUtensorMap tmA, const __grid_constant__ CUtensorMap tmB, const __grid_constant__ GemmParams p) {
   extern __shared__ __align__(1024) uint8_t smem_raw[];
   uint8_t* smem = reinterpret_cast<uint8_t*>((reinterpret_cast<uintptr_t>(smem_raw) + 1023) & ~(uintptr_t)1023);
   constexpr int A_BYTES = BM * BK * 2, B_BYTES = BN * BK * 2;
+  constexpr int MS = BM / 128;
+  static_assert(BM == 128 || (BM == 256 && MODE != 3), "256-row tiles: staged epilogues only (split-K tiles are 128 rows)");
   static_assert(B_BYTES % 1024 == 0, "stage bases must stay 1024-byte aligned for SWIZZLE_128B");
   static_assert(BN % 32 == 0 && BN >= 64 && BN <= 256, "tile width: a multiple of 32 (GEGLU chunks, 32-column epilogue reads)");
-  static_assert(BM * acc_ld(BN) * 4 <= STAGES * (A_BYTES + B_BYTES), "the accumulator tile must fit in the operand ring");
+  static_assert(EPI_ROWS * acc_ld(BN) * 4 <= STAGES * (A_BYTES + B_BYTES), "the accumulator rows must fit in the operand ring");
   constexpr int CSPLIT = col_split(BN);
   uint8_t* sA = smem;
   uint8_t* sB = smem + STAGES * A_BYTES;
@@ -638,35 +648,46 @@
   pdl_wait();
   pdl_trigger();
   if (threadIdx.x == 0) stamp(p, 1);
-
-  const int tiles_m = (p.M + BM - 1) / BM, tiles = tiles_m * ((p.N + BN - 1) / BN);
+  const int tiles_m = (p.M + BM - 1) / BM, tiles_n = (p.N + BN - 1) / BN, tiles = tiles_m * tiles_n;
   const bool persist = MODE != 3 && p.persist;
+  const bool n_fastest = MODE != 3 && p.n_fastest;
+  auto tile_m0 = [&](int t) { return (n_fastest ? t / tiles_n : t % tiles_m) * BM; };
+  auto tile_n0 = [&](int t) { return (n_fastest ? t % tiles_n : t / tiles_m) * BN; };
+  const int t_first = persist ? blockIdx.x : blockIdx.y * tiles_m + blockIdx.x, t_step = persist ? gridDim.x : tiles;
   uint32_t cnt = 0;
-  for (int t = persist ? blockIdx.x : blockIdx.y * tiles_m + blockIdx.x; t < tiles; t += persist ? gridDim.x : tiles) {
-  const int m0 = (t % tiles_m) * BM, n0 = (t / tiles_m) * BN;
   if (warp < 4) {
-    if (threadIdx.x == 0) {
-      asm volatile("fence.proxy.async.shared::cta;" ::: "memory");
-      for (int kb = kb0; kb < kb1; ++kb) {
-        const uint32_t c = cnt + (kb - kb0);
-        const int s = c % STAGES;
-        const uint32_t ph = (c / STAGES) & 1;
-        mbar_wait(empty + s, ph ^ 1, p, WAIT_EMPTY, s);
-        produce_stage<BN>(p, &tmA, &tmB, sA + s * A_BYTES, sB + s * B_BYTES, full + s, kb, m0, n0, bz);
-        if (kb == kb0) stamp(p, 2);
-      }
-      stamp(p, 3);
-    }
-    __syncwarp();
+    reg_dealloc<PRODUCER_REGS>();
+    for (int t = t_first; t < tiles; t += t_step) {
+      const int m0 = tile_m0(t), n0 = tile_n0(t);
+      if (threadIdx.x == 0) {
+        asm volatile("fence.proxy.async.shared::cta;" ::: "memory");
+        for (int kb = kb0; kb < kb1; ++kb) {
+          const uint32_t c = cnt + (kb - kb0);
+          const int s = c % STAGES;
+          const uint32_t ph = (c / STAGES) & 1;
+          mbar_wait(empty + s, ph ^ 1, p, WAIT_EMPTY, s);
+          produce_stage<BM, BN>(p, &tmA, &tmB, sA + s * A_BYTES, sB + s * B_BYTES, full + s, kb, m0, n0, bz);
+          if (kb == kb0) stamp(p, 2);
+        }
+        stamp(p, 3);
+      }
+      __syncwarp();
+      cnt += kb1 - kb0;
+      __syncthreads();
+    }
+    if (split) cluster_sync_all();
   } else {
+    reg_alloc<CONSUMER_REGS>();
     const int wg = (warp >> 2) - 1, e = warp - 4, quarter = e & 3, te = threadIdx.x - 128;
     const int c_lo = e < 4 ? 0 : CSPLIT, c_hi = e < 4 ? CSPLIT : BN;
-    const int row0 = m0 + quarter * 32;
-    if (MODE != 3) epilogue_preload<BN>(p, m0, n0, sbias, srb, te);
-    {
-      float d[BN / 2];
-#pragma unroll
-      for (int i = 0; i < BN / 2; ++i) d[i] = 0.f;
+    for (int t = t_first; t < tiles; t += t_step) {
+      const int m0 = tile_m0(t), n0 = tile_n0(t);
+      if (MODE != 3) epilogue_preload<BM, BN>(p, m0, n0, sbias, srb, te);
+      float d[MS][BN / 2];
+#pragma unroll
+      for (int h = 0; h < MS; ++h)
+#pragma unroll
+        for (int i = 0; i < BN / 2; ++i) d[h][i] = 0.f;
       for (int kb = kb0; kb < kb1; ++kb) {
         const uint32_t c = cnt + (kb - kb0);
         const int s = c % STAGES;
@@ -677,7 +698,9 @@
         wg::fence();
 #pragma unroll
         for (int k = 0; k < BK / 16; ++k)
-          wg::mma_f16<BN>(d, wg::desc_sw128(a0 + k * 32), wg::desc_sw128(b0 + k * 32), 1);
+#pragma unroll
+          for (int h = 0; h < MS; ++h)
+            wg::mma_f16<BN>(d[h], wg::desc_sw128(a0 + h * (2 * 64 * 128) + k * 32), wg::desc_sw128(b0 + k * 32), 1);
         wg::commit();
         wg::wait<1>();
         if (kb > kb0 && (threadIdx.x & 127) == 0) mbar_arrive(empty + (c - 1) % STAGES);
@@ -685,47 +708,49 @@
       wg::wait<0>();
       if ((threadIdx.x & 127) == 0) mbar_arrive(empty + (cnt + kb1 - kb0 - 1) % STAGES);
       if (te == 0) stamp(p, 5);
-      epi_bar();
-      acc_store<BN>(acc, d, 64 * wg, threadIdx.x & 127);
-    }
-    epi_bar();
-    if (te == 0) stamp(p, 6);
-    const float* acc_row = acc + (quarter * 32 + lane) * acc_ld(BN);
-    if (MODE != 3) {
-      const WarpOut g = warp_out<MODE>(p, n0, c_lo, c_hi);
-      uint4 resq[RES_PREFETCH];
-      prefetch_residual(p, g, lane, row0, resq);
-      epilogue_staged<BN, MODE>(p, g, acc_row, slabs + e * 32 * (CSPLIT * 2 + 16), lane, m0, row0, n0, c_lo, c_hi, sbias, srb, resq);
-    } else {
-      const int row = row0 + lane;
-      if (split) {
-        if (te == 0) stamp_ns(p, 17);
+#pragma unroll
+      for (int h = 0; h < MS; ++h) {
+        epi_bar();
+        acc_store<BN>(acc, d[h], 64 * wg, threadIdx.x & 127);
+        epi_bar();
+        if (te == 0 && h == 0) stamp(p, 6);
+        const float* acc_row = acc + (quarter * 32 + lane) * acc_ld(BN);
+        const int row0 = m0 + EPI_ROWS * h + quarter * 32;
+        if (MODE != 3) {
+          const WarpOut g = warp_out<MODE>(p, n0, c_lo, c_hi);
+          uint4 resq[RES_PREFETCH];
+          prefetch_residual(p, g, lane, row0, resq);
+          epilogue_staged<BM, BN, MODE>(p, g, acc_row, slabs + e * 32 * (CSPLIT * 2 + 16), lane, m0, row0, n0, c_lo, c_hi, sbias, srb,
+                                        resq);
+        } else {
+          const int row = row0 + lane;
+          if (split) {
+            if (te == 0) stamp_ns(p, 17);
 #pragma unroll 1
-        for (int c0 = c_lo; c0 < c_hi; c0 += 32) {
-          uint32_t r[32];
-          acc_ld32(acc_row + c0, r);
-          if (row < p.M) splitk_partial(p, r, bz, row, n0 + c0);
+            for (int c0 = c_lo; c0 < c_hi; c0 += 32) {
+              uint32_t r[32];
+              acc_ld32(acc_row + c0, r);
+              if (row < p.M) splitk_partial(p, r, bz, row, n0 + c0);
+            }
+            if (te == 0) stamp_ns(p, 18);
+          } else {
+            const int64_t crow = (p.batched ? (int64_t)(bz % p.nh) * p.stride_c_h + (int64_t)(bz / p.nh) * p.stride_c_b : 0) +
+                                 out_row(p, row < p.M ? row : 0) * p.ldc;
+#pragma unroll 1
+            for (int c0 = c_lo; c0 < c_hi; c0 += 32) {
+              uint32_t r[32];
+              acc_ld32(acc_row + c0, r);
+              if (row < p.M) epilogue_chunk(p, r, row, crow, n0 + c0);
+            }
+          }
         }
-        if (te == 0) stamp_ns(p, 18);
-      } else {
-        const int64_t crow = (p.batched ? (int64_t)(bz % p.nh) * p.stride_c_h + (int64_t)(bz / p.nh) * p.stride_c_b : 0) +
-                             out_row(p, row < p.M ? row : 0) * p.ldc;
-#pragma unroll 1
-        for (int c0 = c_lo; c0 < c_hi; c0 += 32) {
-          uint32_t r[32];
-          acc_ld32(acc_row + c0, r);
-          if (row < p.M) epilogue_chunk(p, r, row, crow, n0 + c0);
-        }
-      }
-    }
-    if (te == 0) stamp(p, 7);
-  }
-  cnt += kb1 - kb0;
-  __syncthreads();
-  }
-  if (split) {
-    cluster_sync_all();
-    if (warp >= 4) {
+      }
+      if (te == 0) stamp(p, 7);
+      cnt += kb1 - kb0;
+      __syncthreads();
+    }
+    if (split) {
+      cluster_sync_all();
       if (threadIdx.x == 128) stamp_ns(p, 21, true);
       splitk_finalize<BN>(p, blockIdx.x * BM, blockIdx.y * BN, bz, threadIdx.x - 128, reinterpret_cast<float*>(smem));
       if (threadIdx.x == 128) stamp_ns(p, 22, true);
@@ -787,7 +812,7 @@
 }
 
 struct Config {
-  int bn, splits;
+  int bm, bn, splits;
   int persist;
 };
 
@@ -802,32 +827,41 @@
 }
 
 float g_model[7] = {40.f, 0.5f, 6300.f, 5.f, 3.f, 4.f, 1.f};
-float predict_us(int M, int N, int nk, int bn, int splits) {
+float predict_us(int M, int N, int nk, int bm, int bn, int splits) {
   const float bw_sm = g_model[0], alpha = g_model[1], cap = g_model[2], fixed = g_model[3], epi = g_model[4], so0 = g_model[5],
               so1 = g_model[6], cyc_per_us = 1750.f;
-  const int tiles = cdiv(M, BM) * cdiv(N, bn);
+  const int tiles = cdiv(M, bm) * cdiv(N, bn);
   const int n = tiles * splits;
   const int kb = cdiv(nk, splits);
-  const float bytes_cta = (float)kb * (float)(BM * BK * 2 + bn * BK * 2);
+  const float bytes_cta = (float)kb * (float)(bm * BK * 2 + bn * BK * 2);
   const int sms = sm_count();
   const int rounds = cdiv(n, sms);
   float f = (float)(n - sms) / (float)sms;
   f = f < 0.f ? 0.f : (f > 1.f ? 1.f : f);
   const float t_sm = (float)rounds * bytes_cta / (bw_sm * (1.f + alpha * f));
   const float t_fabric = (float)n * bytes_cta / cap;
-  const float t_mma = (float)rounds * (float)kb * 4.f * (float)bn;
+  const float t_mma = (float)rounds * (float)kb * 4.f * (float)bn * (float)(bm / 128);
   float t = t_sm > t_fabric ? t_sm : t_fabric;
   if (t_mma > t) t = t_mma;
-  float us = fixed + t / cyc_per_us + epi * (float)bn / 160.f * (float)cdiv(n, sms);
+  float us = fixed + t / cyc_per_us + epi * (float)bn / 160.f * (float)(bm / 128) * (float)cdiv(n, sms);
   if (splits > 1) us += so0 + so1 * (float)splits * (float)bn / 128.f;
   return us;
 }
+
+bool staged_ok(const GemmParams& p) {
+  const int nout = p.act == 3 ? p.N / 2 : p.N;
+  return !p.out_f32 && !p.batched && (nout % 8) == 0 && (p.ldc % 8) == 0 && ((uintptr_t)p.C % 16) == 0 &&
+         (!p.residual || ((uintptr_t)p.residual % 16) == 0);
+}
+
+bool conv_tiles(int H, int W, int bm);
 
 Config pick_config(const GemmParams& p, int nk, bool can_split, int64_t ws_floats) {
   read_force_env();
   Config c;
   const int M = p.M, N = p.N;
   c.persist = 0;
+  c.bm = 128;
   if (p.batched) {
     c.bn = N <= 64 ? 64 : 128, c.splits = 1;
     return c;
@@ -836,58 +870,63 @@
   static const int kSplits[6] = {1, 2, 3, 4, 6, 8};
   const bool split_ok = can_split && p.act != 3 && p.ws && 2 * (int64_t)M * N <= ws_floats;
   const int max_planes = split_ok ? (int)(ws_floats / ((int64_t)M * N)) : 1;
+  const bool tall_ok = staged_ok(p) && (!p.conv || conv_tiles(p.cH, p.cW, 256));
   float best = 1e30f;
   c.bn = 128, c.splits = 1;
-  for (int bi = 0; bi < 4; ++bi) {
-    const int bn = kBn[bi];
-    if (bn > 64 && N <= 64) continue;
-    if (g_force[1] > 0 && bn != g_force[1]) continue;
-    for (int si = 0; si < 6; ++si) {
-      const int sp = kSplits[si];
-      if (g_force[2] > 0 && sp != (g_force[2] > nk ? nk : g_force[2])) continue;
-      if (sp > 1 && (!split_ok || sp > max_planes || sp > MAX_CLUSTER || nk / sp < 3)) continue;
-      const float us = predict_us(M, N, nk, bn, sp);
-      if (us < best) best = us, c.bn = bn, c.splits = sp;
+  for (int bm = 128; bm <= 256; bm += 128) {
+    if (bm == 256 && !tall_ok) continue;
+    if ((g_force[0] == 128 || g_force[0] == 256) && bm != g_force[0]) continue;
+    for (int bi = 0; bi < 4; ++bi) {
+      const int bn = kBn[bi];
+      if (bn > 64 && N <= 64) continue;
+      if (bm == 256 && bn != 128 && bn != 160) continue;
+      if (g_force[1] > 0 && bn != g_force[1]) continue;
+      for (int si = 0; si < 6; ++si) {
+        const int sp = kSplits[si];
+        if (g_force[2] > 0 && sp != (g_force[2] > nk ? nk : g_force[2])) continue;
+        if (sp > 1 && (bm != 128 || !split_ok || sp > max_planes || sp > MAX_CLUSTER || nk / sp < 3)) continue;
+        const float us = predict_us(M, N, nk, bm, bn, sp);
+        if (us < best) best = us, c.bm = bm, c.bn = bn, c.splits = sp;
+      }
     }
   }
   if (best > 1e29f) {
+    c.bm = 128;
     c.bn = (g_force[1] == 64 || g_force[1] == 128 || g_force[1] == 160 || g_force[1] == 256) ? g_force[1] : 128;
     c.splits = 1;
   }
-  const int tiles = cdiv(M, BM) * cdiv(N, c.bn);
+  const int tiles = cdiv(M, c.bm) * cdiv(N, c.bn);
   const int min_tiles = g_persist_min_tiles > 0 ? g_persist_min_tiles : 4 * sm_count();
   c.persist = c.splits == 1 && (g_persist == 1 || (g_persist == 0 && tiles >= min_tiles));
   return c;
 }
 
 int pick_mode(const GemmParams& p, const Config& c) {
-  const int nout = p.act == 3 ? p.N / 2 : p.N;
-  const bool staged = !p.out_f32 && c.splits <= 1 && !p.batched && (nout % 8) == 0 && (p.ldc % 8) == 0 && ((uintptr_t)p.C % 16) == 0 &&
-                      (!p.residual || ((uintptr_t)p.residual % 16) == 0);
-  if (!staged) return 3;
+  if (c.splits > 1 || !staged_ok(p)) return 3;
   return p.act == 0 ? 0 : (p.act == 3 ? 1 : 2);
 }
 
 long long* g_trace = nullptr;
 
-template <int BN, int STAGES, int MODE>
+template <int BM, int BN, int STAGES, int MODE>
 int launch(const CUtensorMap& a, const CUtensorMap& b, GemmParams p, int batch, int persist, cudaStream_t st) {
-  constexpr int SMEM = smem_bytes(BN, STAGES);
+  constexpr int SMEM = smem_bytes(BM, BN, STAGES);
   static_assert(SMEM <= 227 * 1024, "one CTA per SM");
   static PerDeviceOnce attr;
   if (attr.need())
-    O2345_CUDA(cudaFuncSetAttribute(gemm_tc_kernel<BN, STAGES, MODE>, cudaFuncAttributeMaxDynamicSharedMemorySize, SMEM));
-  p.bn = BN, p.mode = MODE;
+    O2345_CUDA(cudaFuncSetAttribute(gemm_tc_kernel<BM, BN, STAGES, MODE>, cudaFuncAttributeMaxDynamicSharedMemorySize, SMEM));
+  p.bm = BM, p.bn = BN, p.mode = MODE;
   p.diag = diag_buffer(st);
   const int splits = (MODE == 3 && batch == 0 && p.splits > 1) ? p.splits : 1;
   p.splits = splits;
   dim3 grid(cdiv(p.M, BM), cdiv(p.N, BN), batch > 0 ? batch : splits);
   p.persist = MODE != 3 && batch == 0 && splits == 1 && persist;
+  p.n_fastest = MODE != 3 && batch == 0 && p.M > p.N;
   if (p.persist) {
     const int tiles = (int)grid.x * (int)grid.y;
     grid = dim3(tiles < sm_count() ? tiles : sm_count(), 1, 1);
   }
-  O2345_CUDA(launch_pdl_cluster(gemm_tc_kernel<BN, STAGES, MODE>, grid, dim3(GEMM_THREADS), (size_t)SMEM, st, 1, splits, a, b, p));
+  O2345_CUDA(launch_pdl_cluster(gemm_tc_kernel<BM, BN, STAGES, MODE>, grid, dim3(GEMM_THREADS), (size_t)SMEM, st, 1, splits, a, b, p));
   O2345_LAUNCH_CHECK();
   return O2345_OK;
 }
@@ -895,10 +934,21 @@
 template <int BN, int STAGES>
 int launch_mode(int mode, const CUtensorMap& a, const CUtensorMap& b, const GemmParams& p, int batch, int persist, cudaStream_t st) {
   switch (mode) {
-    case 0: return launch<BN, STAGES, 0>(a, b, p, batch, persist, st);
-    case 1: return launch<BN, STAGES, 1>(a, b, p, batch, persist, st);
-    case 2: return launch<BN, STAGES, 2>(a, b, p, batch, persist, st);
-    default: return launch<BN, STAGES, 3>(a, b, p, batch, persist, st);
+    case 0: return launch<128, BN, STAGES, 0>(a, b, p, batch, persist, st);
+    case 1: return launch<128, BN, STAGES, 1>(a, b, p, batch, persist, st);
+    case 2: return launch<128, BN, STAGES, 2>(a, b, p, batch, persist, st);
+    default: return launch<128, BN, STAGES, 3>(a, b, p, batch, persist, st);
+  }
+}
+template <int BN, int STAGES>
+int launch_mode_tall(int mode, const CUtensorMap& a, const CUtensorMap& b, const GemmParams& p, int persist, cudaStream_t st) {
+  switch (mode) {
+    case 0: return launch<256, BN, STAGES, 0>(a, b, p, 0, persist, st);
+    case 1: return launch<256, BN, STAGES, 1>(a, b, p, 0, persist, st);
+    case 2: return launch<256, BN, STAGES, 2>(a, b, p, 0, persist, st);
+    default:
+      set_error("o2345_gemm_f16: internal error, a 256-row tile was planned for the generic epilogue");
+      return O2345_EUNSUPPORTED;
   }
 }
 
@@ -907,6 +957,10 @@
     set_error("o2345_gemm_f16: column statistics need the staged fp16 epilogue (16-byte aligned C / residual) or split-K");
     return O2345_EUNSUPPORTED;
   }
+  if (c.bm == 256) {
+    if (c.bn == 128) return launch_mode_tall<128, 3>(mode, a, b, p, c.persist, st);
+    return launch_mode_tall<160, 3>(mode, a, b, p, c.persist, st);
+  }
   if (c.bn == 64) return launch_mode<64, 6>(mode, a, b, p, batch, c.persist, st);
   if (c.bn == 128) return launch_mode<128, 5>(mode, a, b, p, batch, c.persist, st);
   if (c.bn == 160) return launch_mode<160, 4>(mode, a, b, p, batch, c.persist, st);
@@ -917,7 +971,7 @@
   p.bias = nullptr, p.rowbias = nullptr, p.rowbias_ld = 0, p.rows_per_group = 1, p.residual = nullptr;
   p.out_f32 = 0, p.act = 0, p.alpha = 1.f, p.trace = g_trace;
   p.colstats = nullptr, p.stats_rpg = 1, p.stats_groups = 0;
-  p.diag = nullptr, p.bn = p.mode = 0;
+  p.diag = nullptr, p.bm = p.bn = p.mode = 0;
   if (!ep) return O2345_OK;
   O2345_CHECK_ARG(ep->act >= 0 && ep->act <= 4, "unknown activation");
   O2345_CHECK_ARG(!ep->rowbias || (ep->rows_per_group > 0 && (ep->rowbias_ld % 8) == 0 && ((uintptr_t)ep->rowbias % 16) == 0),
@@ -946,9 +1000,9 @@
 
 extern "C" void o2345_debug_gemm_trace(long long* device_buf16) { g_trace = device_buf16; }
 
-extern "C" void o2345_debug_gemm_force(int ctas, int bn, int splits) {
+extern "C" void o2345_debug_gemm_force(int bm, int bn, int splits) {
   read_force_env();
-  g_force[0] = ctas, g_force[1] = bn, g_force[2] = splits;
+  g_force[0] = bm, g_force[1] = bn, g_force[2] = splits;
 }
 
 
@@ -966,9 +1020,9 @@
   static const char* names[] = {"?", "empty (producer waiting for the MMA to free a stage)", "full (MMA issuer waiting for TMA bytes)",
                                 };
   snprintf(buf, n,
-           "gemm_tc_kernel<BN=%d, MODE=%d> M=%d N=%d K=%d conv=%d splits=%d: CTA (%d,%d,%d) rank %d gave up after 4 s "
+           "gemm_tc_kernel<BM=%d, BN=%d, MODE=%d> M=%d N=%d K=%d conv=%d splits=%d: CTA (%d,%d,%d) rank %d gave up after 4 s "
            "on barrier '%s' stage %d",
-           d->bn, d->mode, d->M, d->N, d->K, d->conv, d->splits, d->bx, d->by, d->bz, d->rank,
+           d->bm, d->bn, d->mode, d->M, d->N, d->K, d->conv, d->splits, d->bx, d->by, d->bz, d->rank,
            names[d->tag >= 1 && d->tag <= 2 ? d->tag : 0], d->stage);
   return 1;
 }
@@ -979,9 +1033,19 @@
                 float* splitk_ws, int64_t ws_floats, int taps, int tx, int ox, int oy, int up, int upa, int upb, cudaStream_t st) {
   EncodeTiledFn fn = encode_fn();
   if (!fn) { set_error("cuTensorMapEncodeTiled entry point not available"); return O2345_ECUDA; }
-  const int tw = W >= 128 ? 128 : W;
-  const int th = W >= 128 ? 1 : (128 / W < H ? 128 / W : H);
-  const int tb = 128 / (tw * th);
+  GemmParams p;
+  p.M = B * H * W, p.N = N, p.K = taps * C, p.ldc = ldc, p.nh = 1, p.stride_c_h = 0, p.stride_c_b = 0, p.C = out;
+  int rc = fill_epilogue(p, ep, p.M, N, ldc);
+  if (rc) return rc;
+  p.batched = 0, p.conv = 1, p.cC = C, p.cH = H, p.cW = W, p.cblocks = (C + BK - 1) / BK;
+  p.ctaps = taps, p.ctx = tx, p.cox = ox, p.coy = oy, p.up = up, p.upa = upa, p.upb = upb;
+  set_workspace(p, splitk_ws, ws_floats);
+  const Config c = pick_config(p, taps * p.cblocks, true, ws_floats);
+  p.splits = c.splits;
+  const int bm = c.bm;
+  const int tw = W >= bm ? bm : W;
+  const int th = W >= bm ? 1 : (bm / W < H ? bm / W : H);
+  const int tb = bm / (tw * th);
   CUtensorMap ma, mb;
   {
     cuuint64_t dims[4] = {(cuuint64_t)C, (cuuint64_t)W, (cuuint64_t)H, (cuuint64_t)B};
@@ -993,22 +1057,13 @@
                     CU_TENSOR_MAP_FLOAT_OOB_FILL_NONE);
     if (r != CUDA_SUCCESS) { set_error("cuTensorMapEncodeTiled (conv activation) failed with %d", (int)r); return O2345_ECUDA; }
   }
-  GemmParams p;
-  p.M = B * H * W, p.N = N, p.K = taps * C, p.ldc = ldc, p.nh = 1, p.stride_c_h = 0, p.stride_c_b = 0, p.C = out;
-  int rc = fill_epilogue(p, ep, p.M, N, ldc);
-  if (rc) return rc;
-  p.batched = 0, p.conv = 1, p.cC = C, p.cH = H, p.cW = W, p.cblocks = (C + BK - 1) / BK;
-  p.ctaps = taps, p.ctx = tx, p.cox = ox, p.coy = oy, p.up = up, p.upa = upa, p.upb = upb;
-  set_workspace(p, splitk_ws, ws_floats);
-  const Config c = pick_config(p, taps * p.cblocks, true, ws_floats);
-  p.splits = c.splits;
   rc = make_map(&mb, weight, N, taps * (int64_t)C, taps * (int64_t)C, 0, 0, 0, 0, c.bn);
   if (rc) return rc;
   return dispatch(c, pick_mode(p, c), ma, mb, p, 0, st);
 }
 
-bool conv_tiles(int H, int W) {
-  return (W % 128) == 0 || ((128 % W) == 0 && (((int64_t)H * W >= 128 && (H % (128 / W)) == 0) || ((int64_t)H * W < 128 && (128 % (H * W)) == 0)));
+bool conv_tiles(int H, int W, int bm) {
+  return (W % bm) == 0 || ((bm % W) == 0 && (((int64_t)H * W >= bm && (H % (bm / W)) == 0) || ((int64_t)H * W < bm && (bm % (H * W)) == 0)));
 }
 }
 }
@@ -1017,7 +1072,7 @@
                                  const o2345_epilogue* ep, float* splitk_ws, int64_t ws_floats, o2345_stream_t stream) {
   O2345_CHECK_ARG(x && weight && out, "null pointer");
   O2345_CHECK_ARG(B > 0 && H > 0 && W > 0 && C > 0 && (C % 8) == 0 && N > 0, "bad sizes (C must be a multiple of 8)");
-  O2345_CHECK_ARG(conv_tiles(H, W),
+  O2345_CHECK_ARG(conv_tiles(H, W, 128),
                   "implicit 3x3 conv: the image must tile into 128-pixel boxes (W % 128 == 0, or 128 % W == 0 with "
                   "H % (128 / W) == 0, or 128 % (H * W) == 0)");
   O2345_CHECK_ARG(((uintptr_t)x % 16) == 0 && ((uintptr_t)weight % 16) == 0, "operands must be 16-byte aligned");
@@ -1028,7 +1083,7 @@
                                    const o2345_epilogue* ep, float* splitk_ws, int64_t ws_floats, o2345_stream_t stream) {
   O2345_CHECK_ARG(x && weight4 && out, "null pointer");
   O2345_CHECK_ARG(B > 0 && H > 0 && W > 0 && C > 0 && (C % 8) == 0 && N > 0, "bad sizes (C must be a multiple of 8)");
-  O2345_CHECK_ARG(conv_tiles(H, W), "up-sampling conv: the LOW-resolution image must tile into 128-pixel boxes (see o2345_conv3x3_f16)");
+  O2345_CHECK_ARG(conv_tiles(H, W, 128), "up-sampling conv: the LOW-resolution image must tile into 128-pixel boxes (see o2345_conv3x3_f16)");
   O2345_CHECK_ARG(((uintptr_t)x % 16) == 0 && ((uintptr_t)weight4 % 16) == 0, "operands must be 16-byte aligned");
   O2345_CHECK_ARG(!ep || (!ep->residual && !ep->colstats && !ep->rowbias && ep->act != 3),
                   "up-sampling conv: bias / activation epilogues only (no residual, row bias, statistics, GEGLU)");
@@ -1066,7 +1121,7 @@
   const Config c = pick_config(p, cdiv(K, BK), nh == 0, ws_floats);
   p.splits = c.splits;
   CUtensorMap ma, mb;
-  rc = make_map(&ma, A, M, K, lda, nh, nb, stride_a_h, stride_a_b, BM);
+  rc = make_map(&ma, A, M, K, lda, nh, nb, stride_a_h, stride_a_b, c.bm);
   if (rc) return rc;
   rc = make_map(&mb, B, N, K, ldb, nh, nb, stride_b_h, stride_b_b, c.bn);
   if (rc) return rc;
diff --git a/one-2-3-45_b200/o2345/_lib.py b/one-2-3-45_b200/o2345/_lib.py
--- a/one-2-3-45_b200/o2345/_lib.py
+++ b/one-2-3-45_b200/o2345/_lib.py
@@ -124,7 +124,7 @@
 }
 
 EXPORTED = tuple(_SIGS)
-ABI_VERSION = 5
+ABI_VERSION = 6
 _lib = None
 
 
```

Result: faster. 2.634 (median of 6 runs) (-4.6%).
